# Doubiiu/ToonCrafter

Hardware: AMD Instinct MI355X
Metric: interpolated frames/sec, 512x320x16f DDIM-50 (higher is better)
Workload: dtype bf16; 1 GPU; ToonCrafter_512 320x512x16f ddim_steps=50 CFG 7.5 bf16, 1 clip per GPU (BASELINE.json configs[1]); sampler + 16f decode + 14f re-decode + splice; a different clip every step; parallelism=dp1 (independent clips, one RCCL gather)

## Files before the change

### include/tooncrafter_hip.h

```cpp
#ifndef TOONCRAFTER_HIP_H
#define TOONCRAFTER_HIP_H

#include <stdint.h>

#ifdef __cplusplus
extern "C" {
#endif

#define TC_ABI_VERSION 14

enum {
  TC_OK = 0,
  TC_EINVAL = -1,
  TC_EALIGN = -2,
  TC_ESHAPE = -3,
  TC_EWORKSPACE = -4
};

typedef uint16_t tc_bf16;

enum { TC_ACT_NONE = 0, TC_ACT_SILU = 1, TC_ACT_GELU = 2, TC_ACT_GEGLU = 3 };

enum {
  TC_GATHER_LINEAR = 0,
  TC_GATHER_CONV3x3 = 1,
  TC_GATHER_CONVT3 = 2
};

typedef struct TcGemmParams {
  const tc_bf16* a;
  const tc_bf16* w;
  void* c;
  const float* bias;
  const float* row_bias;
  const tc_bf16* residual;
  int32_t m, n, k;
  int32_t lda, ldw, ldc, ldr;
  int32_t ldrb;
  int32_t row_div;
  float alpha, out_scale;
  int32_t act;
  int32_t out_f32;
  int32_t gather;
  int32_t cin;
  int32_t frames;
  int32_t t_len;
  int32_t h_out, w_out;
  int32_t h_in, w_in;
  int32_t stride;
  int32_t upsample;
  int32_t pad;
  int32_t batch;
  int64_t stride_a, stride_w, stride_c;
  void* workspace;
  int64_t workspace_bytes;
  int32_t a_norm;
  float a_norm_eps;
  float* gn_part;
} TcGemmParams;

int tc_gemm_bf16(const TcGemmParams* p, void* stream);
int64_t tc_gemm_workspace(const TcGemmParams* p);
int tc_gemm_ws_eligible(const TcGemmParams* p);
int tc_gemm_gn_rows(const TcGemmParams* p);

typedef struct TcGemmMxParams {
  TcGemmParams g;
  const uint8_t* a_scale;
  const uint8_t* w_scale;
  int32_t lda_s, ldw_s;
} TcGemmMxParams;
int tc_gemm_mxfp8(const TcGemmMxParams* p, void* stream);
int tc_quant_mxfp8(const tc_bf16* x, int64_t rows, int32_t k, int32_t ld, uint8_t* q, int32_t ldq,
                   uint8_t* s, int32_t lds, void* stream);
int tc_layernorm_mxfp8(const tc_bf16* x, uint8_t* q, int32_t ldq, uint8_t* s, int32_t lds, const float* gamma,
                       const float* beta, int32_t rows, int32_t c, float eps, void* stream);

typedef struct TcFfParams {
  const tc_bf16* x; const tc_bf16* w1; const float* b1; const tc_bf16* w2; const float* b2; tc_bf16* out;
  int32_t m, c, hidden, ldx, ldo, ln;
  float ln_eps;
} TcFfParams;
int tc_ff_geglu_fused_eligible(const TcFfParams* p);
int tc_ff_geglu_fused(const TcFfParams* p, void* stream);

typedef struct TcTbParams {
  const tc_bf16* x; const tc_bf16* wqkv; const float* bqkv; const tc_bf16* wo; const float* bo; tc_bf16* out;
  int32_t b, t, hw, c, heads, ldx, ldo, ln;
  float ln_eps, scale;
} TcTbParams;
int tc_temporal_attn_fused_eligible(const TcTbParams* p);
int tc_temporal_attn_fused(const TcTbParams* p, void* stream);

typedef struct TcTqaParams {
  const tc_bf16* x; const tc_bf16* wqkv; const float* bqkv; tc_bf16* out;
  int32_t b, t, hw, c, heads, ldx, ldo;
  float scale;
} TcTqaParams;
int tc_temporal_qkv_attn_eligible(const TcTqaParams* p);
int tc_temporal_qkv_attn(const TcTqaParams* p, void* stream);

typedef struct TcAttnParams {
  const tc_bf16* q; const tc_bf16* k; const tc_bf16* v; tc_bf16* o;
  int32_t batch, heads, lq, lk;
  int64_t q_sb, k_sb, v_sb, o_sb;
  int32_t q_ss, k_ss, v_ss, o_ss;
  int32_t kv_bdiv;
  int32_t accumulate;
  float scale;
  const tc_bf16* k2; const tc_bf16* v2;
  int32_t lk2, kv2_bdiv;
  int64_t k2_sb, v2_sb;
  int32_t k2_ss, v2_ss;
} TcAttnParams;

int tc_attn_d64(const TcAttnParams* p, void* stream);

typedef struct TcAttnQ8Params {
  const tc_bf16* q; const tc_bf16* k; const tc_bf16* v; tc_bf16* o;
  int32_t batch, heads, lq, lk;
  int64_t q_sb, k_sb, v_sb, o_sb;
  int32_t q_ss, k_ss, v_ss, o_ss;
  float scale;
  void* workspace;
  int64_t workspace_bytes;
} TcAttnQ8Params;
int64_t tc_attn_q8_workspace(const TcAttnQ8Params* p);
int tc_attn_q8_quant_kv(const TcAttnQ8Params* p, void* stream);
int tc_attn_d64_q8(const TcAttnQ8Params* p, void* stream);

#define TC_TEMPORAL_MAX_FRAMES 64
int tc_attn_temporal(const tc_bf16* qkv, tc_bf16* out, int32_t b, int32_t t, int32_t hw,
                     int32_t heads, float scale, void* stream);

int64_t tc_groupnorm_workspace(int32_t samples, int32_t rows, int32_t c);
int tc_groupnorm(const tc_bf16* x, tc_bf16* y, const float* gamma, const float* beta,
                 int32_t samples, int32_t rows, int32_t c, float eps, int32_t silu,
                 void* workspace, int64_t workspace_bytes, void* stream);
int tc_groupnorm_part(const tc_bf16* x, tc_bf16* y, const float* gamma, const float* beta, const float* part,
                      int32_t part_rows, int32_t samples, int32_t rows, int32_t c, float eps, int32_t silu,
                      void* workspace, int64_t workspace_bytes, void* stream);


int tc_layernorm(const tc_bf16* x, tc_bf16* y, const float* gamma, const float* beta,
                 int32_t rows, int32_t c, float eps, void* stream);

#define TC_PREFETCH_MAX 4
typedef struct TcPrefetch {
  const void* ptr[TC_PREFETCH_MAX];
  int64_t bytes[TC_PREFETCH_MAX];
  int32_t n;
} TcPrefetch;
int tc_groupnorm_pf(const tc_bf16* x, tc_bf16* y, const float* gamma, const float* beta,
                    int32_t samples, int32_t rows, int32_t c, float eps, int32_t silu,
                    void* workspace, int64_t workspace_bytes, const TcPrefetch* prefetch, void* stream);
int tc_layernorm_pf(const tc_bf16* x, tc_bf16* y, const float* gamma, const float* beta,
                    int32_t rows, int32_t c, float eps, const TcPrefetch* prefetch, void* stream);

int tc_softmax_rows(const float* s, tc_bf16* p, int32_t rows, int32_t n, int32_t n_out, int32_t lds, int32_t ldo,
                    int32_t causal_period, void* stream);

int tc_nchw_to_rows(const float* x0, int32_t c0, const float* x1, int32_t c1, tc_bf16* out,
                    int32_t c_pad, int32_t b, int32_t t, int32_t hw, float scale, void* stream);
int tc_rows_to_nchw(const void* src, int32_t src_f32, int32_t ld, float* out, int32_t c,
                    int32_t b, int32_t t, int32_t hw, void* stream);
int tc_concat_rows(const tc_bf16* a, int32_t ca, const tc_bf16* b, int32_t cb, tc_bf16* out,
                   int64_t rows, void* stream);

int tc_timestep_embedding(const float* t, tc_bf16* out, int32_t n, int32_t dim, int32_t ld, void* stream);
int tc_silu_f32_to_bf16(const float* x, tc_bf16* y, int64_t n, void* stream);
int tc_timestep_embedding_i64(const int64_t* t, tc_bf16* out, int32_t n, int32_t dim, int32_t ld, void* stream);

int tc_repeat_rows(const void* src, void* dst, int64_t rows, int32_t row_bytes, int32_t n, void* stream);

int tc_time_mix3(const float* rows, int32_t ld, const float* w, const float* bias, float* out,
                 int32_t b, int32_t t, int32_t hw, void* stream);

int tc_video_to_u8(const float* x, uint8_t* out, int32_t b, int32_t t, int32_t hw, void* stream);

typedef struct TcDdimParams {
  const float* x;
  const float* e_cond;
  const float* e_uncond;
  const float* noise;
  float* x_prev; float* pred_x0;
  int32_t b; int64_t n;
  float cfg_scale, guidance_rescale;
  float sqrt_ac, sqrt_1m_ac, sqrt_a_prev, dir_coef , sigma, x0_rescale;
  const float* e_uncond_img;
  float cfg_img;
} TcDdimParams;

int64_t tc_ddim_workspace(int32_t b);
int tc_ddim_step(const TcDdimParams* p, void* workspace, int64_t workspace_bytes, void* stream);

int tc_ddim_step_eps(const TcDdimParams* p, void* workspace, int64_t workspace_bytes, void* stream);

typedef struct TcDdimBlendParams {
  const float* x;
  const float* x0;
  const float* noise;
  const float* mask;
  float* out;
  int32_t b; int64_t n;
  float sqrt_ac, sqrt_1m_ac;
} TcDdimBlendParams;
int tc_ddim_blend(const TcDdimBlendParams* p, void* stream);

int tc_abi_version(void);
const char* tc_build_info(void);

// ... 5 lines not shown
```

### tooncrafter_amd/_lib.py

```python
from __future__ import annotations

import ctypes as C
import os

HERE = os.path.dirname(os.path.abspath(__file__))
LIB_PATH = os.path.join(HERE, "libtooncrafter_hip.so")

TC_ABI_VERSION = 14
TC_TEMPORAL_MAX_FRAMES = 64
ACT_NONE, ACT_SILU, ACT_GELU, ACT_GEGLU = 0, 1, 2, 3
GATHER_LINEAR, GATHER_CONV3x3, GATHER_CONVT3 = 0, 1, 2

ERRORS = {-1: "TC_EINVAL (null pointer / bad size)", -2: "TC_EALIGN (16-byte alignment)",
          -3: "TC_ESHAPE (unsupported shape)", -4: "TC_EWORKSPACE (workspace too small)"}


class TcGemmParams(C.Structure):
    _fields_ = [
        ("a", C.c_void_p), ("w", C.c_void_p), ("c", C.c_void_p),
        ("bias", C.c_void_p), ("row_bias", C.c_void_p), ("residual", C.c_void_p),
        ("m", C.c_int32), ("n", C.c_int32), ("k", C.c_int32),
        ("lda", C.c_int32), ("ldw", C.c_int32), ("ldc", C.c_int32), ("ldr", C.c_int32),
        ("ldrb", C.c_int32), ("row_div", C.c_int32),
        ("alpha", C.c_float), ("out_scale", C.c_float),
        ("act", C.c_int32), ("out_f32", C.c_int32),
        ("gather", C.c_int32), ("cin", C.c_int32), ("frames", C.c_int32), ("t_len", C.c_int32),
        ("h_out", C.c_int32), ("w_out", C.c_int32), ("h_in", C.c_int32), ("w_in", C.c_int32),
        ("stride", C.c_int32), ("upsample", C.c_int32), ("pad", C.c_int32),
        ("batch", C.c_int32),
        ("stride_a", C.c_int64), ("stride_w", C.c_int64), ("stride_c", C.c_int64),
        ("workspace", C.c_void_p), ("workspace_bytes", C.c_int64),
        ("a_norm", C.c_int32), ("a_norm_eps", C.c_float),
        ("gn_part", C.c_void_p),
    ]


class TcGemmMxParams(C.Structure):
    _fields_ = [("g", TcGemmParams), ("a_scale", C.c_void_p), ("w_scale", C.c_void_p),
                ("lda_s", C.c_int32), ("ldw_s", C.c_int32)]


class TcAttnParams(C.Structure):
    _fields_ = [
        ("q", C.c_void_p), ("k", C.c_void_p), ("v", C.c_void_p), ("o", C.c_void_p),
        ("batch", C.c_int32), ("heads", C.c_int32), ("lq", C.c_int32), ("lk", C.c_int32),
        ("q_sb", C.c_int64), ("k_sb", C.c_int64), ("v_sb", C.c_int64), ("o_sb", C.c_int64),
        ("q_ss", C.c_int32), ("k_ss", C.c_int32), ("v_ss", C.c_int32), ("o_ss", C.c_int32),
        ("kv_bdiv", C.c_int32), ("accumulate", C.c_int32), ("scale", C.c_float),
        ("k2", C.c_void_p), ("v2", C.c_void_p), ("lk2", C.c_int32), ("kv2_bdiv", C.c_int32),
        ("k2_sb", C.c_int64), ("v2_sb", C.c_int64), ("k2_ss", C.c_int32), ("v2_ss", C.c_int32),
    ]


class TcAttnQ8Params(C.Structure):
    _fields_ = [
        ("q", C.c_void_p), ("k", C.c_void_p), ("v", C.c_void_p), ("o", C.c_void_p),
        ("batch", C.c_int32), ("heads", C.c_int32), ("lq", C.c_int32), ("lk", C.c_int32),
        ("q_sb", C.c_int64), ("k_sb", C.c_int64), ("v_sb", C.c_int64), ("o_sb", C.c_int64),
        ("q_ss", C.c_int32), ("k_ss", C.c_int32), ("v_ss", C.c_int32), ("o_ss", C.c_int32),
        ("scale", C.c_float),
        ("workspace", C.c_void_p), ("workspace_bytes", C.c_int64),
    ]


class TcDdimParams(C.Structure):
    _fields_ = [
        ("x", C.c_void_p), ("e_cond", C.c_void_p), ("e_uncond", C.c_void_p), ("noise", C.c_void_p),
        ("x_prev", C.c_void_p), ("pred_x0", C.c_void_p),
        ("b", C.c_int32), ("n", C.c_int64),
        ("cfg_scale", C.c_float), ("guidance_rescale", C.c_float),
        ("sqrt_ac", C.c_float), ("sqrt_1m_ac", C.c_float), ("sqrt_a_prev", C.c_float),
        ("dir_coef", C.c_float), ("sigma", C.c_float), ("x0_rescale", C.c_float),
        ("e_uncond_img", C.c_void_p), ("cfg_img", C.c_float),
    ]


class TcDdimBlendParams(C.Structure):
    _fields_ = [
        ("x", C.c_void_p), ("x0", C.c_void_p), ("noise", C.c_void_p), ("mask", C.c_void_p), ("out", C.c_void_p),
        ("b", C.c_int32), ("n", C.c_int64),
        ("sqrt_ac", C.c_float), ("sqrt_1m_ac", C.c_float),
    ]


class TcFfParams(C.Structure):
    _fields_ = [
# ... 21 lines not shown
    ]


TC_PREFETCH_MAX = 4


class TcPrefetch(C.Structure):
    _fields_ = [("ptr", C.c_void_p * TC_PREFETCH_MAX), ("bytes", C.c_int64 * TC_PREFETCH_MAX), ("n", C.c_int32)]


SYMBOLS = {
    "tc_gemm_bf16": (C.c_int, [C.POINTER(TcGemmParams), C.c_void_p]),
    "tc_gemm_workspace": (C.c_int64, [C.POINTER(TcGemmParams)]),
    "tc_gemm_mxfp8": (C.c_int, [C.POINTER(TcGemmMxParams), C.c_void_p]),
    "tc_quant_mxfp8": (C.c_int, [C.c_void_p, C.c_int64, C.c_int32, C.c_int32, C.c_void_p, C.c_int32, C.c_void_p, C.c_int32,
                                 C.c_void_p]),
    "tc_layernorm_mxfp8": (C.c_int, [C.c_void_p, C.c_void_p, C.c_int32, C.c_void_p, C.c_int32, C.c_void_p, C.c_void_p,
                                     C.c_int32, C.c_int32, C.c_float, C.c_void_p]),
    "tc_attn_d64": (C.c_int, [C.POINTER(TcAttnParams), C.c_void_p]),
    "tc_attn_q8_workspace": (C.c_int64, [C.POINTER(TcAttnQ8Params)]),
    "tc_attn_q8_quant_kv": (C.c_int, [C.POINTER(TcAttnQ8Params), C.c_void_p]),
    "tc_attn_d64_q8": (C.c_int, [C.POINTER(TcAttnQ8Params), C.c_void_p]),
    "tc_attn_temporal": (C.c_int, [C.c_void_p, C.c_void_p, C.c_int32, C.c_int32, C.c_int32, C.c_int32,
                                   C.c_float, C.c_void_p]),
    "tc_groupnorm_workspace": (C.c_int64, [C.c_int32, C.c_int32, C.c_int32]),
    "tc_groupnorm": (C.c_int, [C.c_void_p, C.c_void_p, C.c_void_p, C.c_void_p, C.c_int32, C.c_int32, C.c_int32,
                               C.c_float, C.c_int32, C.c_void_p, C.c_int64, C.c_void_p]),
    "tc_layernorm": (C.c_int, [C.c_void_p, C.c_void_p, C.c_void_p, C.c_void_p, C.c_int32, C.c_int32, C.c_float,
                               C.c_void_p]),
    "tc_groupnorm_pf": (C.c_int, [C.c_void_p, C.c_void_p, C.c_void_p, C.c_void_p, C.c_int32, C.c_int32, C.c_int32,
                                  C.c_float, C.c_int32, C.c_void_p, C.c_int64, C.POINTER(TcPrefetch), C.c_void_p]),
    "tc_layernorm_pf": (C.c_int, [C.c_void_p, C.c_void_p, C.c_void_p, C.c_void_p, C.c_int32, C.c_int32, C.c_float,
                                  C.POINTER(TcPrefetch), C.c_void_p]),
    "tc_softmax_rows": (C.c_int, [C.c_void_p, C.c_void_p, C.c_int32, C.c_int32, C.c_int32, C.c_int32, C.c_int32,
                                  C.c_int32, C.c_void_p]),
    "tc_nchw_to_rows": (C.c_int, [C.c_void_p, C.c_int32, C.c_void_p, C.c_int32, C.c_void_p, C.c_int32, C.c_int32,
                                  C.c_int32, C.c_int32, C.c_float, C.c_void_p]),
    "tc_rows_to_nchw": (C.c_int, [C.c_void_p, C.c_int32, C.c_int32, C.c_void_p, C.c_int32, C.c_int32, C.c_int32,
                                  C.c_int32, C.c_void_p]),
    "tc_concat_rows": (C.c_int, [C.c_void_p, C.c_int32, C.c_void_p, C.c_int32, C.c_void_p, C.c_int64, C.c_void_p]),
    "tc_timestep_embedding": (C.c_int, [C.c_void_p, C.c_void_p, C.c_int32, C.c_int32, C.c_int32, C.c_void_p]),
    "tc_silu_f32_to_bf16": (C.c_int, [C.c_void_p, C.c_void_p, C.c_int64, C.c_void_p]),
    "tc_timestep_embedding_i64": (C.c_int, [C.c_void_p, C.c_void_p, C.c_int32, C.c_int32, C.c_int32, C.c_void_p]),
    "tc_repeat_rows": (C.c_int, [C.c_void_p, C.c_void_p, C.c_int64, C.c_int32, C.c_int32, C.c_void_p]),
    "tc_time_mix3": (C.c_int, [C.c_void_p, C.c_int32, C.c_void_p, C.c_void_p, C.c_void_p, C.c_int32, C.c_int32,
                               C.c_int32, C.c_void_p]),
    "tc_video_to_u8": (C.c_int, [C.c_void_p, C.c_void_p, C.c_int32, C.c_int32, C.c_int32, C.c_void_p]),
    "tc_ddim_workspace": (C.c_int64, [C.c_int32]),
    "tc_ddim_step": (C.c_int, [C.POINTER(TcDdimParams), C.c_void_p, C.c_int64, C.c_void_p]),
    "tc_ddim_step_eps": (C.c_int, [C.POINTER(TcDdimParams), C.c_void_p, C.c_int64, C.c_void_p]),
    "tc_ddim_blend": (C.c_int, [C.POINTER(TcDdimBlendParams), C.c_void_p]),
    "tc_gemm_ws_eligible": (C.c_int, [C.POINTER(TcGemmParams)]),
    "tc_gemm_gn_rows": (C.c_int, [C.POINTER(TcGemmParams)]),
    "tc_groupnorm_part": (C.c_int, [C.c_void_p, C.c_void_p, C.c_void_p, C.c_void_p, C.c_void_p, C.c_int32, C.c_int32, C.c_int32,
                                    C.c_int32, C.c_float, C.c_int32, C.c_void_p, C.c_int64, C.c_void_p]),
    "tc_ff_geglu_fused_eligible": (C.c_int, [C.POINTER(TcFfParams)]),
    "tc_ff_geglu_fused": (C.c_int, [C.POINTER(TcFfParams), C.c_void_p]),
    "tc_temporal_attn_fused_eligible": (C.c_int, [C.POINTER(TcTbParams)]),
    "tc_temporal_attn_fused": (C.c_int, [C.POINTER(TcTbParams), C.c_void_p]),
    "tc_temporal_qkv_attn_eligible": (C.c_int, [C.POINTER(TcTqaParams)]),
    "tc_temporal_qkv_attn": (C.c_int, [C.POINTER(TcTqaParams), C.c_void_p]),
    "tc_abi_version": (C.c_int, []),
    "tc_build_info": (C.c_char_p, []),
}

_lib = None


class TooncrafterHipError(RuntimeError):
    pass


class TooncrafterAbiError(TooncrafterHipError):
    """A library built against another ABI version was loaded: a stale build, never a reason to fall back."""


def load():
    global _lib
    if _lib is not None:
        return _lib
    if not os.path.exists(LIB_PATH):
        raise TooncrafterHipError(
            f"{LIB_PATH} not found: build it with `python -m tooncrafter_amd.build` "
            "(hipcc --offload-arch=gfx950). There is no fallback path.")
    lib = C.CDLL(LIB_PATH)
    for name, (res, args) in SYMBOLS.items():
        fn = getattr(lib, name)
        fn.restype = res
        fn.argtypes = args
    ver = lib.tc_abi_version()
    if ver != TC_ABI_VERSION:
        raise TooncrafterHipError(f"ABI mismatch: library {ver}, binding {TC_ABI_VERSION}")
    if os.environ.get("TC_DEBUG_SYNC"):
        lib = _TracedLib(lib)
    _lib = lib
    return lib


class _TracedLib:

    def __init__(self, lib):
        self._lib = lib

    def __getattr__(self, name):
        fn = getattr(self._lib, name)
        if name not in SYMBOLS or name in ("tc_abi_version", "tc_build_info") or name.endswith("_workspace"):
# ... 31 lines not shown
```

### tooncrafter_amd/csrc/gemm.hip

```cpp
#include "gemm_common.h"
#include "gemm_epilogue.h"

#include <stdio.h>

namespace {

constexpr int BK = TC_BK;

template <int GATHER, int TM, int TN, bool PIPE>
__global__ __launch_bounds__(256, 2) void gemm_kernel(const TcGemmParams pin, const int splits, const int order,
                                                      const int late_epi) {
  TcGemmParams p = pin;
  if (splits > 1) {
    p.c = reinterpret_cast<float*>(pin.workspace) + (int64_t)blockIdx.y * pin.m * pin.n;
    p.ldc = pin.n;
    p.out_f32 = 1;
    p.bias = nullptr; p.row_bias = nullptr; p.residual = nullptr;
    p.act = TC_ACT_NONE; p.alpha = 1.f; p.out_scale = 1.f;
  }
  constexpr int BM = 64 * TM, BN = 64 * TN;
  constexpr int STAGE_BYTES = (BM + BN) * BK * 2;
  constexpr int EPI_BYTES = BM * BN * 4;
  constexpr int SMEM_BYTES = 2 * STAGE_BYTES > EPI_BYTES ? 2 * STAGE_BYTES : EPI_BYTES;
  constexpr int RA = BM / 32, RB = BN / 32;
  __shared__ __attribute__((aligned(1024))) char smem[SMEM_BYTES];

  const int tid = threadIdx.x;
  const int lane = tid & 63;
  const int wave = tid >> 6;
  const int wm = wave >> 1, wn = wave & 1;
  const int wave_u = __builtin_amdgcn_readfirstlane(wave);

  const int tiles_n = (p.n + BN - 1) / BN;
  const int tiles_m = (p.m + BM - 1) / BM;
  int tile_m, tile_n;
  tc_tile_of_block(blockIdx.x, tiles_m, tiles_n, order, tile_m, tile_n);
  if (tile_m >= tiles_m) return;

  const int64_t bz = blockIdx.z;
  const tc_rsrc_t w_rsrc = make_rsrc(reinterpret_cast<const bf16_t*>(p.w) + bz * p.stride_w, tc_w_extent(p));

  const int lrow = tid >> 3;
  const int chunk = (tid & 7) ^ ((lrow >> 1) & 7);
  AGather<GATHER, RA> ag;
  ag.init(p, tile_m * BM, lrow, 32, chunk);
  const tc_rsrc_t a_rsrc = tc_a_rsrc(p, bz, ag.row_lo);
  uint32_t b_voff[RB];
#pragma unroll
  for (int i = 0; i < RB; ++i) {
    const int n = tile_n * BN + lrow + 32 * i;
    b_voff[i] = n < p.n ? (uint32_t)((int64_t)n * p.ldw * 2 + chunk * 16) : TC_OOB;
  }
  const bool k_ragged = (p.k & (BK - 1)) != 0;
#if defined(TC_ABLATE) && (TC_ABLATE & 2)
  const int kb_first = blockIdx.y * (((p.k + BK - 1) / BK + splits - 1) / splits);
#endif

  auto load_tile = [&](int kb, int stage) {
#if defined(TC_ABLATE) && (TC_ABLATE & 2)
    if (kb >= kb_first + 2) return;
#endif
    const int k0 = kb * BK;
    uint32_t a_voff[RA], a_soff;
    ag.offsets(p, k0, chunk, a_voff, a_soff);
    const uint32_t kill = (k_ragged && (k0 + chunk * 8 >= p.k)) ? TC_OOB : 0u;
    char* sa = smem + stage * STAGE_BYTES + wave_u * 1024;
    char* sb = sa + BM * BK * 2;
#pragma unroll
    for (int i = 0; i < RB; ++i)
      glds16(w_rsrc, sb + i * 4096, b_voff[i] | kill, (uint32_t)k0 * 2u);
#pragma unroll
    for (int i = 0; i < RA; ++i)
      glds16(a_rsrc, sa + i * 4096, a_voff[i] | kill, a_soff);
  };

  f32x16 acc[TM][TN];
#pragma unroll
  for (int i = 0; i < TM; ++i)
#pragma unroll
    for (int j = 0; j < TN; ++j)
#pragma unroll
      for (int r = 0; r < 16; ++r) acc[i][j][r] = 0.f;

  const int frow = lane & 31;
  const int fhalf = lane >> 5;

  auto compute = [&](int stage) {
    const char* sa = smem + stage * STAGE_BYTES;
    const char* sb = sa + BM * BK * 2;
    bf16x8 af[2][TM], bf[2][TN];
    auto frags = [&](int kk, bf16x8 (&a)[TM], bf16x8 (&b)[TN]) {
      const int c = kk * 2 + fhalf;
#pragma unroll
      for (int i = 0; i < TM; ++i)
        a[i] = *reinterpret_cast<const bf16x8*>(sa + lds_off(wm * 32 * TM + i * 32 + frow, c));
#pragma unroll
      for (int j = 0; j < TN; ++j)
        b[j] = *reinterpret_cast<const bf16x8*>(sb + lds_off(wn * 32 * TN + j * 32 + frow, c));
    };
    auto mfmas = [&](bf16x8 (&a)[TM], bf16x8 (&b)[TN]) {
#if defined(TC_ABLATE) && (TC_ABLATE & 1)
      asm volatile("" ::"v"(a[0]), "v"(b[0]));
      return;
#endif
#pragma unroll
      for (int i = 0; i < TM; ++i)
#pragma unroll
        for (int j = 0; j < TN; ++j)
          acc[i][j] = __builtin_amdgcn_mfma_f32_32x32x16_bf16(a[i], b[j], acc[i][j], 0, 0, 0);
    };
    frags(0, af[0], bf[0]);
    frags(1, af[1], bf[1]);
    __builtin_amdgcn_sched_barrier(0);
    mfmas(af[0], bf[0]);
    __builtin_amdgcn_sched_barrier(0);
    frags(2, af[0], bf[0]);
    __builtin_amdgcn_sched_barrier(0);
    mfmas(af[1], bf[1]);
    __builtin_amdgcn_sched_barrier(0);
    frags(3, af[1], bf[1]);
    __builtin_amdgcn_sched_barrier(0);
    mfmas(af[0], bf[0]);
    mfmas(af[1], bf[1]);
// ... 83 lines not shown
    }
  }
  else if (p.alpha == 1.f && p.out_scale == 1.f && p.act == TC_ACT_NONE && !p.row_bias)
    epilogue_fast<false, BM, BN, true>(p, cs, tid, tile_m, tile_n, bz, pre);
  else epilogue_fast<false, BM, BN, false>(p, cs, tid, tile_m, tile_n, bz, pre);
}

__global__ __launch_bounds__(256) void splitk_reduce_kernel(const TcGemmParams p, const int splits) {
  const int vpr = p.n >> 3;
  const int64_t v = (int64_t)blockIdx.x * 256 + threadIdx.x;
  if (v >= (int64_t)p.m * vpr) return;
  const int m = (int)(v / vpr), n0 = (int)(v - (int64_t)m * vpr) * 8;
  const float* ws = reinterpret_cast<const float*>(p.workspace) + (int64_t)m * p.n + n0;
  float x[8] = {0.f, 0.f, 0.f, 0.f, 0.f, 0.f, 0.f, 0.f};
  for (int s = 0; s < splits; ++s) {
    const f32x4 lo = *reinterpret_cast<const f32x4*>(ws + (int64_t)s * p.m * p.n);
    const f32x4 hi = *reinterpret_cast<const f32x4*>(ws + (int64_t)s * p.m * p.n + 4);
#pragma unroll
    for (int e = 0; e < 4; ++e) { x[e] += lo[e]; x[4 + e] += hi[e]; }
  }
#pragma unroll
  for (int e = 0; e < 8; ++e) {
    float t = x[e] * p.alpha;
    if (p.bias) t += p.bias[n0 + e];
    if (p.row_bias) t += p.row_bias[(int64_t)(m / p.row_div) * p.ldrb + n0 + e];
    x[e] = apply_act(t, p.act) * p.out_scale;
  }
  if (p.residual) {
    float rf[8];
    unpack8(*reinterpret_cast<const u32x4*>(reinterpret_cast<const bf16_t*>(p.residual) + (int64_t)m * p.ldr + n0), rf);
#pragma unroll
    for (int e = 0; e < 8; ++e) x[e] += rf[e];
  }
  if (p.out_f32) {
    float* op = reinterpret_cast<float*>(p.c) + (int64_t)m * p.ldc + n0;
    *reinterpret_cast<f32x4*>(op) = f32x4{x[0], x[1], x[2], x[3]};
    *reinterpret_cast<f32x4*>(op + 4) = f32x4{x[4], x[5], x[6], x[7]};
  } else {
    *reinterpret_cast<u32x4*>(reinterpret_cast<bf16_t*>(p.c) + (int64_t)m * p.ldc + n0) = pack8(x);
  }
}

}

static void tc_gemm_tile_launch(const TcGemmParams& p, const TcGemmRoute& r, hipStream_t s) {
  const dim3 grid(r.grid[0], r.grid[1], r.grid[2]), block(r.block);
  const auto go = [&](auto g, auto pipe) {
    constexpr int G = decltype(g)::value, P = decltype(pipe)::value;
    if (r.tm == 2 && r.tn == 2) hipLaunchKernelGGL((gemm_kernel<G, 2, 2, P>), grid, block, 0, s, p, r.splits, r.order, r.late_epi);
    else if (r.tm == 2) hipLaunchKernelGGL((gemm_kernel<G, 2, 1, P>), grid, block, 0, s, p, r.splits, r.order, r.late_epi);
    else if (r.tn == 2) hipLaunchKernelGGL((gemm_kernel<G, 1, 2, P>), grid, block, 0, s, p, r.splits, r.order, r.late_epi);
    else hipLaunchKernelGGL((gemm_kernel<G, 1, 1, P>), grid, block, 0, s, p, r.splits, r.order, r.late_epi);
  };
  tc_with_gather(p.gather, [&](auto g) { if (r.pipe) go(g, std::true_type{}); else go(g, std::false_type{}); });
}

extern "C" int tc_gemm_bf16(const TcGemmParams* pp, void* stream) {
  if (!pp) return TC_EINVAL;
  const TcGemmParams& p = *pp;
  if (const int rc = tc_gemm_validate(p)) return rc;
  const int cus = tc_cu_count();
  const TcGemmSwitches sw = tc_gemm_switches();
  TcGemmRoute r;
  const int rc = tc_gemm_route(p, sw, cus, &r);
  static bool said = false;
  if (r.halo_yielded && !said) {
    said = true;
    fprintf(stderr, "[tooncrafter_hip] %s=%s is set: the 3x3 convolutions stay on the implicit-GEMM kernels "
                    "(halo-patch route suppressed; TC_CONV_HALO=2 forces it)\n", sw.forcing_name, sw.forcing_value);
  }
  if (rc != TC_OK) return rc;
  static TcGemmLaunch* const launch[] = {tc_gemm_ws_launch, tc_conv_halo_launch, tc_gemm8_launch, tc_gemm_tile16_launch,
                                         tc_gemm_wide_launch, tc_gemm_tile_launch};
  launch[r.family](p, r, reinterpret_cast<hipStream_t>(stream));
  TC_LAUNCH_CHECK();
  if (r.family == TC_FAM_TILE && r.splits > 1) {
    const int64_t vecs = (int64_t)p.m * (p.n >> 3);
    hipLaunchKernelGGL(splitk_reduce_kernel, dim3((unsigned)((vecs + 255) / 256)), dim3(256), 0, reinterpret_cast<hipStream_t>(stream), p, r.splits);
    TC_LAUNCH_CHECK();
  }
  return TC_OK;
}
```

### tooncrafter_amd/csrc/gemm_mx.hip

```cpp
#include "gemm_common.h"
#include "gemm_epilogue.h"
#include "mx_quant.h"

namespace {

constexpr int BKE = 128;
typedef int i32x8 __attribute__((ext_vector_type(8)));
typedef int i32x4 __attribute__((ext_vector_type(4)));

template <int GATHER, int R>
struct MxRows {
  uint32_t base[R];
  uint32_t vbits[R];
  int f[R], y[R], x[R];
  bool ok[R];

  __device__ __forceinline__ void init(const TcGemmParams& p, int ld, int row0, int row_step) {
    const int hw = p.h_out * p.w_out;
#pragma unroll
    for (int i = 0; i < R; ++i) {
      const int mm = row0 + row_step * i;
      ok[i] = mm < p.m;
      const int mc = ok[i] ? mm : 0;
      f[i] = y[i] = x[i] = 0;
// ... 248 lines not shown
  const u32x4* src = reinterpret_cast<const u32x4*>(x + row * ld + blk * 32);
  u32x4 v[4];
#pragma unroll
  for (int i = 0; i < 4; ++i) v[i] = src[i];
  uint32_t amax = 0;
#pragma unroll
  for (int i = 0; i < 4; ++i)
#pragma unroll
    for (int e = 0; e < 4; ++e) {
      const uint32_t lo = v[i][e] & 0x7fffu, hi = (v[i][e] >> 16) & 0x7fffu;
      amax = max(amax, max(lo, hi));
    }
  const int byte = mx_scale_byte(amax);
  const float inv = mx_inv_scale(byte);
  uint32_t out[8];
#pragma unroll
  for (int i = 0; i < 4; ++i) {
    float f[8];
    unpack8(v[i], f);
    out[i * 2] = mx_quant4(f[0], f[1], f[2], f[3], inv);
    out[i * 2 + 1] = mx_quant4(f[4], f[5], f[6], f[7], inv);
  }
  u32x4* dst = reinterpret_cast<u32x4*>(q + row * ldq + blk * 32);
  dst[0] = u32x4{out[0], out[1], out[2], out[3]};
  dst[1] = u32x4{out[4], out[5], out[6], out[7]};
  s[slot] = (uint8_t)byte;
}

}

extern "C" int tc_quant_mxfp8(const tc_bf16* x, int64_t rows, int32_t k, int32_t ld, uint8_t* q, int32_t ldq,
                              uint8_t* s, int32_t lds, void* stream) {
  if (!x || !q || !s || rows <= 0 || k <= 0) return TC_EINVAL;
  if ((k & 31) || (ld & 7) || (ldq & 15) || !tc_aligned16(x) || !tc_aligned16(q)) return TC_EALIGN;
  if (ld < k || ldq < k || lds * 32 < k) return TC_ESHAPE;
  const int64_t slots = rows * lds;
  if ((slots + 255) / 256 > 0x7fffffffLL) return TC_ESHAPE;
  hipLaunchKernelGGL(quant_mx_kernel, dim3((unsigned)((slots + 255) / 256)), dim3(256), 0, reinterpret_cast<hipStream_t>(stream),
                     reinterpret_cast<const bf16_t*>(x), rows, k, ld, q, ldq, s, lds);
  TC_LAUNCH_CHECK();
  return TC_OK;
}

extern "C" int tc_gemm_mxfp8(const TcGemmMxParams* pp, void* stream) {
  if (!pp) return TC_EINVAL;
  const TcGemmParams& p = pp->g;
  if (!p.a || !p.w || !p.c || !pp->a_scale || !pp->w_scale || p.m <= 0 || p.n <= 0 || p.k <= 0) return TC_EINVAL;
  if (!tc_aligned16(p.a) || !tc_aligned16(p.w) || !tc_aligned16(p.c)) return TC_EALIGN;
  if (p.residual && !tc_aligned16(p.residual)) return TC_EALIGN;
  if ((p.k & 31) || (p.lda & 15) || (p.ldw & 15)) return TC_EALIGN;
  if ((reinterpret_cast<uintptr_t>(pp->a_scale) & 1u) || (reinterpret_cast<uintptr_t>(pp->w_scale) & 3u)) return TC_EALIGN;
  if ((pp->lda_s & 1) || (pp->ldw_s & 3)) return TC_EALIGN;
  if (p.ldw < p.k || pp->ldw_s < ((p.k + 127) / 128) * 4) return TC_ESHAPE;
  if ((p.batch > 1) || p.stride_a || p.stride_w || p.stride_c) return TC_ESHAPE;
  const bool geglu = p.act == TC_ACT_GEGLU;
  const int n_out = geglu ? p.n / 2 : p.n;
  if ((n_out & 7) == 0) {
    if (p.out_f32 ? (p.ldc & 3) : (p.ldc & 7)) return TC_EALIGN;
    if (p.residual && (p.ldr & 7)) return TC_EALIGN;
    if (p.bias && (reinterpret_cast<uintptr_t>(p.bias) & 15u)) return TC_EALIGN;
    if (p.row_bias && ((reinterpret_cast<uintptr_t>(p.row_bias) & 15u) || (p.ldrb & 3))) return TC_EALIGN;
  }
  if (p.ldc < n_out || (p.residual && p.ldr < n_out)) return TC_ESHAPE;
  if (geglu && ((p.n % 128) != 0 || p.row_bias || p.residual)) return TC_ESHAPE;
  if (p.row_bias && (p.row_div <= 0 || p.ldrb < p.n)) return TC_EINVAL;
  if (p.act < TC_ACT_NONE || p.act > TC_ACT_GEGLU) return TC_EINVAL;
  if (p.gather == TC_GATHER_LINEAR) {
    if (p.lda < p.k || pp->lda_s < ((p.k + 63) / 64) * 2) return TC_ESHAPE;
  } else if (p.gather == TC_GATHER_CONV3x3 || p.gather == TC_GATHER_CONVT3) {
    const int taps = p.gather == TC_GATHER_CONV3x3 ? 9 : 3;
    if (p.cin <= 0 || (p.cin % 64) != 0 || p.k != taps * p.cin || p.lda < p.cin || pp->lda_s * 32 < p.cin) return TC_ESHAPE;
    if ((int64_t)p.k * p.cin >= (1LL << 32)) return TC_ESHAPE;
    if (p.frames <= 0 || p.h_out <= 0 || p.w_out <= 0) return TC_ESHAPE;
    if ((int64_t)p.frames * p.h_out * p.w_out != p.m) return TC_ESHAPE;
    if (p.gather == TC_GATHER_CONV3x3) {
      if (p.h_in <= 0 || p.w_in <= 0 || (p.stride != 1 && p.stride != 2)) return TC_ESHAPE;
      if (p.upsample && p.stride != 1) return TC_ESHAPE;
      const int hvv = p.upsample ? 2 * p.h_in : p.h_in, wvv = p.upsample ? 2 * p.w_in : p.w_in;
      if (p.pad != 0 && p.pad != 1) return TC_ESHAPE;
      const int extra = p.pad == 1 ? 2 : 1;
      if ((hvv + extra - 3) / p.stride + 1 != p.h_out || (wvv + extra - 3) / p.stride + 1 != p.w_out) return TC_ESHAPE;
    } else {
      if (p.t_len <= 0 || (p.frames % p.t_len) != 0) return TC_ESHAPE;
    }
  } else {
    return TC_EINVAL;
  }
  if (tc_a_rows(p) * p.lda >= 0x7fffff00LL || (int64_t)p.n * p.ldw >= 0x7fffff00LL) return TC_ESHAPE;
  hipStream_t s = reinterpret_cast<hipStream_t>(stream);
  const int64_t big_tiles = (int64_t)((p.n + 127) / 128) * ((p.m + 127) / 128);
  const bool small = !geglu && big_tiles < 384;
  const int bm = small ? 64 : 128;
  const int tiles_n = (p.n + bm - 1) / bm;
  const int tiles_m = (p.m + bm - 1) / bm;
  const int64_t nblk = (int64_t)tiles_n * 8 * ((tiles_m + 7) / 8);
  if (nblk > 0x7fffffffLL) return TC_ESHAPE;
  dim3 grid((unsigned)nblk), block(256);
  TcGemmParams half = p;
  half.ldw = p.ldw / 2;
  const int order = tc_gemm_tile_order(half, tiles_n, tc_gemm_switches());
#define TC_LAUNCH_MX(G)                                                                            \
  do {                                                                                             \
    if (small) hipLaunchKernelGGL((gemm_mx_kernel<G, 1, 1>), grid, block, 0, s, *pp, order);        \
    else hipLaunchKernelGGL((gemm_mx_kernel<G, 2, 2>), grid, block, 0, s, *pp, order);              \
  } while (0)
  switch (p.gather) {
    case TC_GATHER_LINEAR: TC_LAUNCH_MX(TC_GATHER_LINEAR); break;
// ... 8 lines not shown
```

### tooncrafter_amd/csrc/gemm_route.cpp

```cpp
#include "gemm_route.h"

#include <stdlib.h>
#include <string.h>

namespace {

typedef TcGemmSwitches S;
const struct Sw { const char* name; const char* dflt; bool implicit_gemm; char kind; int S::*field; } kSwitches[] = {
    {"TC_GEMM_TILE", nullptr, false, 't', &S::tile},
    {"TC_GEMM_TILE16", "1", true, 'i', &S::tile16},
    {"TC_GEMM8", "1", true, 'i', &S::gemm8},
    {"TC_GEMM_PIPE", "1", true, 'p', &S::pipe},
    {"TC_GEMM_SPLITK", nullptr, true, 'k', &S::splitk},
    {"TC_GEMM_WS", "1", true, 'i', &S::ws},
    {"TC_G16_ILV", nullptr, true, 'l', &S::ilv},
    {"TC_G16_TALL", "0", true, 'i', &S::g16_tall},
    {"TC_GEMM_WIDE", "1", true, '0', &S::wide},
    {"TC_GEMM_ORDER", "8", true, 'i', &S::order},
    {"TC_GEMM_NMAJOR", "1", true, 'i', &S::nmajor},
    {"TC_GEMM_ORDER_MIB", "4", false, 'm', nullptr},
    {"TC_GEMM_EPI_LATE", "0", false, '1', &S::epi_late},
    {"TC_G8_GRID", "0", false, 'i', &S::g8_grid},
    {"TC_G8_STAGGER", "0", false, 'i', &S::g8_stagger},
    {"TC_CONV_HALO", "1", false, 'i', &S::halo},
// ... 8 lines not shown

void take(TcGemmRoute* r, int family, int64_t gx, int gy, int gz, int block) {
  r->family = family, r->block = (unsigned)block;
  r->grid[0] = (unsigned)gx, r->grid[1] = (unsigned)gy, r->grid[2] = (unsigned)gz;
}

}

TcGemmSwitches tc_gemm_switches() {
  TcGemmSwitches s{};
  for (const Sw& sw : kSwitches) {
    const char* e = getenv(sw.name);
    const char* v = e ? e : sw.dflt;
    if (sw.implicit_gemm && !s.forcing_name && e && e[0] && !(sw.dflt && strcmp(e, sw.dflt) == 0)) s.forcing_name = sw.name, s.forcing_value = e;
    if (sw.kind == 'i') s.*sw.field = atoi(v);
    else if (sw.kind == '0') s.*sw.field = v[0] != '0';
    else if (sw.kind == '1') s.*sw.field = v[0] == '1';
    else if (sw.kind == 'p') s.pipe = v[0] == '0' ? 0 : v[0] == '2' ? 2 : 1;
    else if (sw.kind == 'k') s.splitk = e ? atoi(e) : -1;
    else if (sw.kind == 'l') s.ilv_set = e != nullptr, s.ilv = e ? atoi(e) : 0;
    else if (sw.kind == 'm') s.order_bytes = (int64_t)(atof(v) * (1 << 20));
    else if (e) {
      const int t = e[0] == 'w' ? 1 : e[0] == 'b' ? 22 : e[0] == 's' ? 11 : atoi(e);
      s.tile = (t == 22 || t == 21 || t == 12 || t == 11 || e[0] == 'w') ? t : 0, s.tile_set = e[0] != 0;
    }
  }
  static const TcGemmSwitches first = s;
  s.order = first.order, s.order_bytes = first.order_bytes;
  return s;
}

int tc_gemm_tile_order(const TcGemmParams& p, int tiles_n, const TcGemmSwitches& sw) {
  return (sw.order > 0 && tiles_n >= 2 * sw.order && (int64_t)p.n * p.ldw * 2 > sw.order_bytes) ? sw.order : 0;
}

int tc_gemm_validate(const TcGemmParams& p) {
  if (!p.a || !p.w || !p.c || p.m <= 0 || p.n <= 0 || p.k <= 0) return TC_EINVAL;
  if (!aligned16(p.a) || !aligned16(p.w) || !aligned16(p.c)) return TC_EALIGN;
  if (p.residual && !aligned16(p.residual)) return TC_EALIGN;
  if ((p.k & 7) || (p.lda & 7) || (p.ldw & 7)) return TC_EALIGN;
  if (p.ldw < p.k) return TC_ESHAPE;
  const bool geglu = p.act == TC_ACT_GEGLU;
  const int n_out = geglu ? p.n / 2 : p.n;
  if ((n_out & 7) == 0) {
    if (p.out_f32 ? (p.ldc & 3) : (p.ldc & 7)) return TC_EALIGN;
    if (p.residual && (p.ldr & 7)) return TC_EALIGN;
    if (p.bias && !aligned16(p.bias)) return TC_EALIGN;
    if (p.row_bias && (!aligned16(p.row_bias) || (p.ldrb & 3))) return TC_EALIGN;
  }
  if (p.ldc < n_out || (p.residual && p.ldr < n_out)) return TC_ESHAPE;
  if (geglu && ((p.n % 128) != 0 || p.row_bias || p.residual)) return TC_ESHAPE;
  if (p.row_bias && (p.row_div <= 0 || p.ldrb < p.n)) return TC_EINVAL;
  if (p.act < TC_ACT_NONE || p.act > TC_ACT_GEGLU) return TC_EINVAL;
  if (p.gather == TC_GATHER_LINEAR) {
    if (p.lda < p.k) return TC_ESHAPE;
  } else if (p.gather == TC_GATHER_CONV3x3 || p.gather == TC_GATHER_CONVT3) {
    const int taps = p.gather == TC_GATHER_CONV3x3 ? 9 : 3;
    if (p.cin <= 0 || (p.cin % 64) != 0 || p.k != taps * p.cin || p.lda < p.cin) return TC_ESHAPE;
    if (p.frames <= 0 || p.h_out <= 0 || p.w_out <= 0) return TC_ESHAPE;
    if ((int64_t)p.frames * p.h_out * p.w_out != p.m) return TC_ESHAPE;
    if (p.gather == TC_GATHER_CONV3x3) {
      if (p.h_in <= 0 || p.w_in <= 0 || (p.stride != 1 && p.stride != 2)) return TC_ESHAPE;
      if (p.upsample && p.stride != 1) return TC_ESHAPE;
      const int hvv = p.upsample ? 2 * p.h_in : p.h_in, wvv = p.upsample ? 2 * p.w_in : p.w_in;
      if (p.pad != 0 && p.pad != 1) return TC_ESHAPE;
      const int extra = p.pad == 1 ? 2 : 1;
      if ((hvv + extra - 3) / p.stride + 1 != p.h_out || (wvv + extra - 3) / p.stride + 1 != p.w_out) return TC_ESHAPE;
    } else {
      if (p.t_len <= 0 || (p.frames % p.t_len) != 0) return TC_ESHAPE;
    }
  } else {
    return TC_EINVAL;
  }
  int64_t span_rows = 256;
  if (p.gather == TC_GATHER_CONVT3) span_rows += 2 * (int64_t)p.h_out * p.w_out;
  else if (p.gather == TC_GATHER_CONV3x3)
    span_rows = ((int64_t)256 / (p.w_out > 0 ? p.w_out : 1) + 2) * p.stride * p.w_in + 4 * (int64_t)p.w_in + 8;
  const int64_t a_bytes = (span_rows + 1) * p.lda * 2, w_bytes = (int64_t)p.n * p.ldw * 2;
  return (a_bytes < 0x7fffff00LL && w_bytes < 0x7fffff00LL) ? TC_OK : TC_ESHAPE;
}

static bool tc_gemm_ws_takes(const TcGemmParams& p, const TcGemmSwitches& sw, int batch) {
  if (sw.tile_set) return false;
  if (sw.ws == 0 || batch != 1 || p.gather != TC_GATHER_LINEAR || p.k != TC_WS_K || p.lda < TC_WS_K) return false;
  if (p.row_bias || p.alpha != 1.f || p.out_scale != 1.f || p.out_f32) return false;
  const bool geglu = p.act == TC_ACT_GEGLU;
  if (!geglu && p.act != TC_ACT_NONE) return false;
  if (p.n % (geglu ? 256 : 320) != 0) return false;
  if (p.residual && geglu) return false;
  if ((sw.ws == 1 || sw.ws == 5) && (p.m < 65536 || geglu || p.n != 320)) return false;
  if ((int64_t)p.m * p.lda * 2 >= 0x7fffff00LL) return false;
  if ((int64_t)p.m * p.ldc * 2 >= 0x7fffff00LL || (p.residual && (int64_t)p.m * p.ldr * 2 >= 0x7fffff00LL)) return false;
  return true;
}

static void route_ws(const TcGemmParams& p, const TcGemmSwitches& sw, TcGemmRoute* r) {
  r->geglu = p.act == TC_ACT_GEGLU, r->res = p.residual != nullptr, r->ln = p.a_norm != 0;
  const int slabs = p.n / (r->geglu ? 256 : 320);
  const int ntiles = (p.m + TC_WS_ROWS - 1) / TC_WS_ROWS;
  int nchunks = 256 / slabs < 1 ? 1 : 256 / slabs;
  r->nchunks = nchunks = nchunks > ntiles ? ntiles : nchunks;
  r->safe = sw.ws == 3 ? 1 : (sw.ws == 2 ? 0 : 2);
  take(r, TC_FAM_WS, slabs * 8 * ((nchunks + 7) / 8), 1, 1, 256);
}

static int route_halo(const TcGemmParams& p, const TcGemmSwitches& sw, int batch, TcGemmRoute* r) {
  if (sw.halo == 0) return 0;
// ... 133 lines not shown
  const int force = sw.splitk;
  const int batch = p.batch > 0 ? p.batch : 1;
  if (force == 0 || batch != 1 || p.act == TC_ACT_GEGLU || (p.n & 7) != 0) return 1;
  const int nk = (p.k + TC_BK - 1) / TC_BK;
  const int64_t tiles = (int64_t)((p.n + 127) / 128) * ((p.m + 127) / 128);
  if (tiles >= 200 || (force < 0 && nk < 128)) return 1;
  int s = force > 0 ? force : (int)(512 / tiles);
  if (s > 8) s = 8;
  if (s > nk / 8) s = nk / 8;
  if (force <= 0) while (s & (s - 1)) s &= s - 1;
  return s < 2 ? 1 : s;
}

static void pick_tile(int m, int n, int batch, bool geglu, int* tm, int* tn) {
  const int64_t big_tiles = (int64_t)((n + 127) / 128) * ((m + 127) / 128) * batch;
  const bool small = !geglu && big_tiles < 384;
  *tm = small ? 1 : 2;
  *tn = small ? 1 : 2;
  if (!geglu && n <= 64) {
    *tn = 1;
    *tm = m >= 262144 ? 2 : 1;
  }
}

static int route_tile(const TcGemmParams& p, const TcGemmSwitches& sw, int batch, bool gn_ok, TcGemmRoute* r) {
  const bool geglu = p.act == TC_ACT_GEGLU;
  const int force = sw.tile;
  int tm = 2, tn = 2;
  int splits = (p.workspace && force == 0) ? tc_gemm_splits(p, sw) : 1;
  if (splits > 1 && p.workspace_bytes < (int64_t)splits * p.m * p.n * (int64_t)sizeof(float)) splits = 1;
  if (force > 1) {
    tm = force / 10;
    tn = geglu ? 2 : force % 10;
  } else if (splits == 1) {
    pick_tile(p.m, p.n, batch, geglu, &tm, &tn);
  }
  r->gn_rows = (gn_ok && splits == 1 && tm == 2 && tn == 2) ? 128 : 0;
  if (p.gn_part && !r->gn_rows) return TC_ESHAPE;
  if (splits > 1 && !aligned16(p.workspace)) return TC_EALIGN;
  const int bm = 64 * tm, bn = 64 * tn;
  const int tiles_n = (p.n + bn - 1) / bn;
  const int tiles_m = (p.m + bm - 1) / bm;
  const bool nmajor = sw.nmajor != 0 && p.batch <= 1 && (sw.nmajor == 2 || (p.m <= 2048 && tc_w_extent(p) > tc_a_extent(p)));
  const int64_t nblk = nmajor ? 8 * (((int64_t)tiles_m * tiles_n + 7) / 8) : (int64_t)tiles_n * 8 * ((tiles_m + 7) / 8);
  if (nblk > 0x7fffffffLL || batch > 65535) return TC_ESHAPE;
  take(r, TC_FAM_TILE, nblk, splits, batch, 256);
  r->tm = tm, r->tn = tn, r->splits = splits;
  r->order = nmajor ? -1 : tc_gemm_tile_order(p, tiles_n, sw);
  r->pipe = sw.pipe != 0, r->late_epi = sw.epi_late;
  return TC_OK;
}

int tc_gemm_route(const TcGemmParams& p, const TcGemmSwitches& sw, int cus, TcGemmRoute* r) {
  *r = TcGemmRoute{};
  const int batch = p.batch > 0 ? p.batch : 1;
  const bool gn_ok = batch == 1 && p.act != TC_ACT_GEGLU && !p.out_f32 && (p.n & 7) == 0 && !p.a_norm && !sw.tile_set && sw.gn_part;
  if (p.gn_part && !gn_ok) return TC_ESHAPE;
  const auto emits = [&](int rows) {
    r->gn_rows = gn_ok ? rows : 0;
    return (p.gn_part && !r->gn_rows) ? TC_ESHAPE : TC_OK;
  };
  const int force = sw.tile;
  if (force == 0 && tc_gemm_ws_takes(p, sw, batch)) return route_ws(p, sw, r), emits(0);
  if (p.a_norm) return TC_ESHAPE;
  if (force == 0 && !p.gn_part) {
    const int h = route_halo(p, sw, batch, r);
    if (h < 0) return TC_ESHAPE;
    if (h > 0) return TC_OK;
  }
  if (force == 0 && route_gemm8(p, sw, batch, cus, r)) return emits(0);
  if (force == 0 && route_tile16(p, sw, batch, r)) return emits(TC_T16);
  if (force <= 1 && route_wide(p, sw, batch, force == 1, r)) return emits(0);
  return route_tile(p, sw, batch, gn_ok, r);
}

extern "C" int64_t tc_gemm_workspace(const TcGemmParams* p) {
  if (!p || p->m <= 0 || p->n <= 0 || p->k <= 0) return 0;
  const int s = tc_gemm_splits(*p, tc_gemm_switches());
  return s > 1 ? (int64_t)s * p->m * p->n * (int64_t)sizeof(float) : 0;
}
extern "C" int tc_gemm_ws_eligible(const TcGemmParams* p) {
  return (p && tc_gemm_ws_takes(*p, tc_gemm_switches(), p->batch > 0 ? p->batch : 1)) ? 1 : 0;
}

extern "C" int tc_gemm_gn_rows(const TcGemmParams* pp) {
  if (!pp || pp->m <= 0 || pp->n <= 0 || pp->k <= 0) return 0;
  TcGemmParams p = *pp;
  if (!p.gn_part) p.gn_part = reinterpret_cast<float*>(16);
  TcGemmRoute r;
  tc_gemm_route(p, tc_gemm_switches(), 256, &r);
  return r.gn_rows;
}
```

### tooncrafter_amd/csrc/norm.hip

```cpp
#include "common.h"
#include "mx_quant.h"

#include <stdlib.h>

namespace {

constexpr int GN_THREADS = 256;
constexpr int GN_MAX_SLOTS = 2;
constexpr int GN_TARGET_BLOCKS = 512;
constexpr int GN_MIN_ROWS = 8;

constexpr int PF_MAX = 4;
struct PfArgs {
  const u32x4* p[PF_MAX];
  uint32_t units[PF_MAX];
  int n;
};

__device__ __forceinline__ void pf_run(const PfArgs& pf, uint32_t b, uint32_t nb, uint32_t tid, uint32_t nthr) {
#pragma unroll 1
  for (int i = 0; i < pf.n; ++i) {
    const u32x4* src = pf.p[i];
    const uint32_t units = pf.units[i];
    uint32_t per = (units + nb - 1) / nb;
    per = (per + 7u) & ~7u;
    const uint32_t lo = b * per;
    if (lo >= units) continue;
    const uint32_t hi = min(units, lo + per);
#pragma unroll 1
    for (uint32_t u = lo + tid; u < hi; u += nthr * 16u) {
      u32x4 v[16];
#pragma unroll
      for (int k = 0; k < 16; ++k) {
        const uint32_t uu = u + (uint32_t)k * nthr;
        v[k] = uu < hi ? src[uu] : u32x4{0u, 0u, 0u, 0u};
      }
#pragma unroll
      for (int k = 0; k < 16; ++k) asm volatile("" ::"v"(v[k][0]), "v"(v[k][1]), "v"(v[k][2]), "v"(v[k][3]));
    }
  }
}

struct GnGeo {
  int vpr;
  int slots;
  int rows_pp;
};

__host__ __device__ __forceinline__ GnGeo gn_geo(int c) {
  GnGeo g;
  g.vpr = c >> 3;
  g.slots = (g.vpr + GN_THREADS - 1) / GN_THREADS;
  const int vps = (g.vpr + g.slots - 1) / g.slots;
  g.rows_pp = g.slots > 1 ? 1 : GN_THREADS / vps;
  if (g.rows_pp < 1) g.rows_pp = 1;
  return g;
}

__device__ __forceinline__ void gn_thread_map(const GnGeo& g, int tid, int& rlane, int (&vec)[GN_MAX_SLOTS]) {
  if (g.slots > 1) {
    rlane = 0;
#pragma unroll
    for (int s = 0; s < GN_MAX_SLOTS; ++s) {
      const int v = tid + s * GN_THREADS;
      vec[s] = (s < g.slots && v < g.vpr) ? v : -1;
    }
  } else {
    rlane = tid / g.vpr;
    vec[0] = rlane < g.rows_pp ? tid - rlane * g.vpr : -1;
    if (rlane >= g.rows_pp) rlane = 0;
    vec[1] = -1;
  }
}

__global__ __launch_bounds__(GN_THREADS) void gn_stats_kernel(const bf16_t* __restrict__ x, float* __restrict__ part,
                                                              int rows, int c, int nchunks, int chunk_rows) {
  __shared__ float red[2][4096 + 32];
  const GnGeo g = gn_geo(c);
  const int tid = threadIdx.x;
  int rlane, vec[GN_MAX_SLOTS];
  gn_thread_map(g, tid, rlane, vec);
  const int sample = blockIdx.y, chunk = blockIdx.x;
  const int r0 = chunk * chunk_rows;
  const int r1 = min(rows, r0 + chunk_rows);
  const bf16_t* xs = x + (int64_t)sample * rows * c;

  float sum[GN_MAX_SLOTS][8], sq[GN_MAX_SLOTS][8];
#pragma unroll
  for (int s = 0; s < GN_MAX_SLOTS; ++s)
#pragma unroll
    for (int e = 0; e < 8; ++e) { sum[s][e] = 0.f; sq[s][e] = 0.f; }

  const int step = g.rows_pp;
  for (int r = r0 + rlane; r < r1; r += 4 * step) {
#pragma unroll
    for (int s = 0; s < GN_MAX_SLOTS; ++s) {
      if (vec[s] >= 0) {
        u32x4 v4[4];
#pragma unroll
        for (int u = 0; u < 4; ++u) {
          const int rr = r + u * step;
          v4[u] = rr < r1 ? *reinterpret_cast<const u32x4*>(xs + (int64_t)rr * c + vec[s] * 8)
                          : u32x4{0u, 0u, 0u, 0u};
        }
#pragma unroll
        for (int u = 0; u < 4; ++u) {
          float f[8];
          unpack8(v4[u], f);
#pragma unroll
          for (int e = 0; e < 8; ++e) { sum[s][e] += f[e]; sq[s][e] += f[e] * f[e]; }
        }
      }
    }
  }
  for (int pass = 0; pass < g.rows_pp; ++pass) {
    if (rlane == pass) {
#pragma unroll
      for (int s = 0; s < GN_MAX_SLOTS; ++s)
        if (vec[s] >= 0) {
#pragma unroll
          for (int e = 0; e < 8; ++e) {
            const int ch = vec[s] * 8 + e;
            if (pass == 0) { red[0][ch] = sum[s][e]; red[1][ch] = sq[s][e]; }
            else { red[0][ch] += sum[s][e]; red[1][ch] += sq[s][e]; }
          }
        }
    }
    __syncthreads();
  }
  if (tid < 32) {
    const int cpg = c / 32;
    float a = 0.f, b = 0.f;
    for (int i = 0; i < cpg; ++i) { a += red[0][tid * cpg + i]; b += red[1][tid * cpg + i]; }
    float* o = part + (((int64_t)sample * nchunks + chunk) * 32 + tid) * 2;
    o[0] = a;
    o[1] = b;
  }
}

__global__ __launch_bounds__(256) void gn_finalize_kernel(const float* __restrict__ part, float* __restrict__ stats,
                                                          int samples, int rows, int c, int nchunks, float eps) {
  const int lane = threadIdx.x & 63;
  const int sg = blockIdx.x * 4 + (threadIdx.x >> 6);
  if (sg >= samples * 32) return;
  const int sample = sg >> 5, grp = sg & 31;
  const float* pp = part + ((int64_t)sample * nchunks * 32 + grp) * 2;
  double a = 0.0, b = 0.0;
  for (int k = lane; k < nchunks; k += 64) {
    const float2 v = *reinterpret_cast<const float2*>(pp + (int64_t)k * 64);
    a += v.x;
    b += v.y;
  }
#pragma unroll
  for (int off = 32; off > 0; off >>= 1) { a += __shfl_xor(a, off, 64); b += __shfl_xor(b, off, 64); }
  if (lane == 0) {
    const double cnt = (double)rows * (c / 32);
    const double mean = a / cnt;
    double var = b / cnt - mean * mean;
    if (var < 0.0) var = 0.0;
    stats[(int64_t)sg * 2] = (float)mean;
    stats[(int64_t)sg * 2 + 1] = (float)(1.0 / sqrt(var + (double)eps));
  }
}

__global__ __launch_bounds__(256) void gn_finalize_part_kernel(const float* __restrict__ part, float* __restrict__ stats,
                                                               int samples, int rows, int c, int prows, float eps) {
  __shared__ double red[2][4];
  const int tid = threadIdx.x, lane = tid & 63, wave = tid >> 6;
  const int sg = blockIdx.x;
  const int sample = sg >> 5, grp = sg & 31;
  const int cpg = c / 32, nb = rows / prows;
  const float* pp = part + ((int64_t)sample * nb * 2) * c + grp * cpg;
  double a = 0.0, b = 0.0;
  for (int blk = tid; blk < nb; blk += 256) {
    const float* r0 = pp + (int64_t)blk * 2 * c;
    for (int ch = 0; ch < cpg; ++ch) { a += r0[ch]; b += r0[c + ch]; }
  }
#pragma unroll
  for (int off = 32; off > 0; off >>= 1) { a += __shfl_xor(a, off, 64); b += __shfl_xor(b, off, 64); }
  if (lane == 0) { red[0][wave] = a; red[1][wave] = b; }
  __syncthreads();
  if (tid == 0) {
    a = red[0][0] + red[0][1] + red[0][2] + red[0][3];
    b = red[1][0] + red[1][1] + red[1][2] + red[1][3];
    const double cnt = (double)rows * cpg;
    const double mean = a / cnt;
    double var = b / cnt - mean * mean;
    if (var < 0.0) var = 0.0;
    stats[(int64_t)sg * 2] = (float)mean;
    stats[(int64_t)sg * 2 + 1] = (float)(1.0 / sqrt(var + (double)eps));
  }
}

template <bool SILU>
__global__ __launch_bounds__(GN_THREADS) void gn_apply_kernel(const bf16_t* __restrict__ x, bf16_t* __restrict__ y,
                                                              const float* __restrict__ gamma, const float* __restrict__ beta,
                                                              const float* __restrict__ stats, int rows, int c,
                                                              int chunk_rows, const PfArgs pf) {
  if (blockIdx.z) {
    pf_run(pf, ((blockIdx.z - 1) * gridDim.y + blockIdx.y) * gridDim.x + blockIdx.x, (gridDim.z - 1) * gridDim.y * gridDim.x,
           threadIdx.x, GN_THREADS);
    return;
  }
  const GnGeo g = gn_geo(c);
  const int tid = threadIdx.x;
  int rlane, vec[GN_MAX_SLOTS];
  gn_thread_map(g, tid, rlane, vec);
  const int sample = blockIdx.y, chunk = blockIdx.x;
  const float* st = stats + (int64_t)sample * 64;
  const int cpg = c / 32;
  float sc[GN_MAX_SLOTS][8], sh[GN_MAX_SLOTS][8];
#pragma unroll
  for (int s = 0; s < GN_MAX_SLOTS; ++s)
#pragma unroll
    for (int e = 0; e < 8; ++e) {
      sc[s][e] = 0.f; sh[s][e] = 0.f;
      if (vec[s] >= 0) {
        const int ch = vec[s] * 8 + e;
        const int grp = ch / cpg;
        const float a = st[grp * 2 + 1] * gamma[ch];
        sc[s][e] = a;
        sh[s][e] = beta[ch] - st[grp * 2] * a;
      }
    }
  const int r0 = chunk * chunk_rows;
  const int r1 = min(rows, r0 + chunk_rows);
  const bf16_t* xs = x + (int64_t)sample * rows * c;
  bf16_t* ys = y + (int64_t)sample * rows * c;
  const int step = g.rows_pp;
  for (int r = r0 + rlane; r < r1; r += 4 * step) {
#pragma unroll
    for (int s = 0; s < GN_MAX_SLOTS; ++s) {
      if (vec[s] >= 0) {
        u32x4 v4[4];
#pragma unroll
        for (int u = 0; u < 4; ++u) {
          const int rr = r + u * step;
          if (rr < r1) v4[u] = *reinterpret_cast<const u32x4*>(xs + (int64_t)rr * c + vec[s] * 8);
        }
#pragma unroll
        for (int u = 0; u < 4; ++u) {
          const int rr = r + u * step;
          if (rr < r1) {
            float f[8];
            unpack8(v4[u], f);
#pragma unroll
            for (int e = 0; e < 8; ++e) {
              const float v = f[e] * sc[s][e] + sh[s][e];
              f[e] = SILU ? silu_f(v) : v;
            }
            *reinterpret_cast<u32x4*>(ys + (int64_t)rr * c + vec[s] * 8) = pack8(f);
          }
        }
      }
    }
  }
}

__device__ __forceinline__ void gn_opaque(u32x4& v) { asm volatile("" : "+v"(v[0]), "+v"(v[1]), "+v"(v[2]), "+v"(v[3])); }

template <int T, int NV, bool SILU>
__global__ __launch_bounds__(T) void gn_onepass_kernel(const bf16_t* __restrict__ x, bf16_t* __restrict__ y,
                                                       const float* __restrict__ gamma, const float* __restrict__ beta,
                                                       int rows, int c, int vu, float eps, const PfArgs pf) {
  if (blockIdx.z) {
    pf_run(pf, ((blockIdx.z - 1) * gridDim.y + blockIdx.y) * gridDim.x + blockIdx.x, (gridDim.z - 1) * gridDim.y * gridDim.x,
           threadIdx.x, T);
    return;
  }
  constexpr int NW = T / 64;
  __shared__ float red[2][NW][4];
  const int tid = threadIdx.x, lane = tid & 63, wave = tid >> 6;
  const int cpg = c >> 5;
  const int rpp = T / vu;
  const int col = tid % vu, r0 = tid / vu;
  const bool live = tid < rpp * vu;
  const int unit = blockIdx.x, sample = blockIdx.y;
  const int ch0 = (unit * vu + col) * 8;
  const int ug0 = (unit * vu * 8) / cpg;
  const bf16_t* xs = x + (int64_t)sample * rows * c + ch0;
  bf16_t* ys = y + (int64_t)sample * rows * c + ch0;
  int gl[8];
#pragma unroll
  for (int e = 0; e < 8; ++e) gl[e] = (ch0 + e) / cpg - ug0;

  u32x4 v[NV];
#pragma unroll
  for (int i = 0; i < NV; ++i) {
    const int r = r0 + i * rpp;
    v[i] = (live && r < rows) ? *reinterpret_cast<const u32x4*>(xs + (int64_t)r * c) : u32x4{0u, 0u, 0u, 0u};
  }
  auto group_sums = [&](const float (&pc)[8], int slot, float (&out)[4]) {
    float g4[4] = {0.f, 0.f, 0.f, 0.f};
#pragma unroll
    for (int e = 0; e < 8; ++e)
#pragma unroll
      for (int g = 0; g < 4; ++g) g4[g] += (gl[e] == g) ? pc[e] : 0.f;
#pragma unroll
    for (int g = 0; g < 4; ++g) g4[g] = wave_sum(g4[g]);
    if (lane == 0) {
#pragma unroll
      for (int g = 0; g < 4; ++g) red[slot][wave][g] = g4[g];
    }
    __syncthreads();
#pragma unroll
    for (int g = 0; g < 4; ++g) {
      float t = 0.f;
#pragma unroll
      for (int w = 0; w < NW; ++w) t += red[slot][w][g];
      out[g] = t;
    }
  };
  float pc[8] = {0.f, 0.f, 0.f, 0.f, 0.f, 0.f, 0.f, 0.f};
#pragma unroll
  for (int i = 0; i < NV; ++i) {
    float f[8];
    unpack8(v[i], f);
#pragma unroll
    for (int e = 0; e < 8; ++e) pc[e] += f[e];
  }
  float gs[4];
  group_sums(pc, 0, gs);
  const float inv_cnt = 1.0f / ((float)rows * (float)cpg);
  float mean_e[8];
#pragma unroll
  for (int e = 0; e < 8; ++e) {
    float m = 0.f;
#pragma unroll
    for (int g = 0; g < 4; ++g) m = (gl[e] == g) ? gs[g] * inv_cnt : m;
    mean_e[e] = m;
  }
#pragma unroll
  for (int e = 0; e < 8; ++e) pc[e] = 0.f;
#pragma unroll
  for (int i = 0; i < NV; ++i) {
    const int r = r0 + i * rpp;
    gn_opaque(v[i]);
    if (live && r < rows) {
      float f[8];
      unpack8(v[i], f);
#pragma unroll
      for (int e = 0; e < 8; ++e) { const float d = f[e] - mean_e[e]; pc[e] += d * d; }
    }
// ... 154 lines not shown
static int pf_args(const TcPrefetch* pf, PfArgs* out) {
  PfArgs a{};
  a.n = 0;
  if (pf) {
    if (pf->n < 0 || pf->n > TC_PREFETCH_MAX) return TC_EINVAL;
    for (int i = 0; i < pf->n; ++i) {
      if (!pf->ptr[i] || pf->bytes[i] < 0 || pf->bytes[i] > ((int64_t)1 << 35)) return TC_EINVAL;
      if (!tc_aligned16(pf->ptr[i])) return TC_EALIGN;
      const uint32_t units = (uint32_t)(pf->bytes[i] >> 4);
      if (!units) continue;
      a.p[a.n] = reinterpret_cast<const u32x4*>(pf->ptr[i]);
      a.units[a.n] = units;
      ++a.n;
    }
  }
  *out = a;
  return TC_OK;
}
static inline unsigned pf_planes(const PfArgs& a, int64_t plane) {
  if (!a.n || plane <= 0) return 0;
  int64_t z = (512 + plane - 1) / plane;
  if (z > 8) {
    int64_t units = 0;
    for (int i = 0; i < a.n; ++i) units += a.units[i];
    int64_t need = (units * 16 + 65535) / 65536;
    if (need > 512) need = 512;
    const int64_t zn = (need + plane - 1) / plane;
    z = zn > 8 ? (zn > 64 ? 64 : zn) : 8;
  }
  return (unsigned)(z < 1 ? 1 : z);
}

static inline void gn_chunking(int samples, int rows, int* nchunks, int* chunk_rows) {
  static const int target = [] { const char* e = getenv("TC_GN_BLOCKS"); const int v = e ? atoi(e) : 0;
                                 return v > 0 ? v : GN_TARGET_BLOCKS; }();
  int per_sample = target / (samples > 0 ? samples : 1);
  if (per_sample < 1) per_sample = 1;
  int max_chunks = (rows + GN_MIN_ROWS - 1) / GN_MIN_ROWS;
  int n = per_sample < max_chunks ? per_sample : max_chunks;
  if (n < 1) n = 1;
  const int cr = (rows + n - 1) / n;
  *chunk_rows = cr;
  *nchunks = (rows + cr - 1) / cr;
}

extern "C" int64_t tc_groupnorm_workspace(int32_t samples, int32_t rows, int32_t c) {
  (void)c;
  if (samples <= 0 || rows <= 0) return 0;
  int nch, cr;
  gn_chunking(samples, rows, &nch, &cr);
  return ((int64_t)samples * nch * 64 + (int64_t)samples * 64) * sizeof(float);
}

static int gn_check(const tc_bf16* x, tc_bf16* y, const float* gamma, const float* beta, int32_t samples, int32_t rows,
                    int32_t c, void* workspace, int64_t workspace_bytes, const TcPrefetch* prefetch, PfArgs* pf) {
  if (!x || !y || !gamma || !beta || !workspace || samples <= 0 || rows <= 0 || c <= 0) return TC_EINVAL;
  if (const int rc = pf_args(prefetch, pf)) return rc;
  if ((c % 32) != 0 || c > GN_MAX_SLOTS * GN_THREADS * 8 || c > 4096) return TC_ESHAPE;
  if (!tc_aligned16(x) || !tc_aligned16(y)) return TC_EALIGN;
  if (workspace_bytes < tc_groupnorm_workspace(samples, rows, c)) return TC_EWORKSPACE;
  if (samples > 65535) return TC_ESHAPE;
  return TC_OK;
}

struct GnIo {
  const bf16_t* x; bf16_t* y; const float* gamma; const float* beta;
  int rows, c; bool silu; hipStream_t s;
};
static void gn_apply_launch(const GnIo& io, dim3 grid, const float* stats, int chunk_rows, const PfArgs& pf) {
  const auto k = io.silu ? gn_apply_kernel<true> : gn_apply_kernel<false>;
  hipLaunchKernelGGL(k, grid, dim3(GN_THREADS), 0, io.s, io.x, io.y, io.gamma, io.beta, stats, io.rows, io.c, chunk_rows, pf);
}
template <int T, int NV>
static void gn_onepass_launch(const GnIo& io, dim3 grid, int vu, float eps, const PfArgs& pf) {
  const auto k = io.silu ? gn_onepass_kernel<T, NV, true> : gn_onepass_kernel<T, NV, false>;
  hipLaunchKernelGGL(k, grid, dim3(T), 0, io.s, io.x, io.y, io.gamma, io.beta, io.rows, io.c, vu, eps, pf);
}

static int groupnorm_impl(const tc_bf16* x, tc_bf16* y, const float* gamma, const float* beta,
                          int32_t samples, int32_t rows, int32_t c, float eps, int32_t silu,
                          void* workspace, int64_t workspace_bytes, const TcPrefetch* prefetch, void* stream) {
  PfArgs pf;
  if (const int rc = gn_check(x, y, gamma, beta, samples, rows, c, workspace, workspace_bytes, prefetch, &pf)) return rc;
  const GnIo io = {reinterpret_cast<const bf16_t*>(x), reinterpret_cast<bf16_t*>(y), gamma, beta, rows, c, silu != 0,
                   reinterpret_cast<hipStream_t>(stream)};
  {
    static const bool onepass = [] { const char* e = getenv("TC_GN_ONEPASS"); return !(e && e[0] == '0'); }();
    const int cpg = c / 32;
    int u = cpg;
    while (u % 8) u += cpg;
    const int vu = u / 8, gu = u / cpg;
    if (onepass && (c % u) == 0 && gu <= 4 && vu <= 64 && tc_aligned16(gamma) && tc_aligned16(beta)) {
      const int64_t nvec = (int64_t)rows * vu;
      const dim3 grid(c / u, samples, 1 + pf_planes(pf, (int64_t)(c / u) * samples));
      auto fits = [&](int t, int nv) { return (int64_t)((rows + t / vu - 1) / (t / vu)) <= nv; };
      const int64_t nblk = (int64_t)(c / u) * samples;
      const int64_t bytes = nvec * 16 * samples * (c / u);
      bool done = nblk >= 128 || bytes <= (4 << 20);
      if (done && fits(256, 4)) gn_onepass_launch<256, 4>(io, grid, vu, eps, pf);
      else if (done && fits(256, 13)) gn_onepass_launch<256, 13>(io, grid, vu, eps, pf);
      else done = false;
      if (done) {
        TC_LAUNCH_CHECK();
        return TC_OK;
      }
    }
  }
  int nch, cr;
  gn_chunking(samples, rows, &nch, &cr);
  float* part = reinterpret_cast<float*>(workspace);
  float* stats = part + (int64_t)samples * nch * 64;
  dim3 grid(nch, samples), block(GN_THREADS);
  hipLaunchKernelGGL(gn_stats_kernel, grid, block, 0, io.s, io.x, part, rows, c, nch, cr);
  TC_LAUNCH_CHECK();
  hipLaunchKernelGGL(gn_finalize_kernel, dim3((samples * 32 + 3) / 4), block, 0, io.s, part, stats, samples, rows, c, nch,
                     eps);
  TC_LAUNCH_CHECK();
  gn_apply_launch(io, dim3(nch, samples, 1 + pf_planes(pf, (int64_t)nch * samples)), stats, cr, pf);
  TC_LAUNCH_CHECK();
  return TC_OK;
}

extern "C" int tc_groupnorm(const tc_bf16* x, tc_bf16* y, const float* gamma, const float* beta,
                            int32_t samples, int32_t rows, int32_t c, float eps, int32_t silu,
                            void* workspace, int64_t workspace_bytes, void* stream) {
  return groupnorm_impl(x, y, gamma, beta, samples, rows, c, eps, silu, workspace, workspace_bytes, nullptr, stream);
}

extern "C" int tc_groupnorm_pf(const tc_bf16* x, tc_bf16* y, const float* gamma, const float* beta,
                               int32_t samples, int32_t rows, int32_t c, float eps, int32_t silu,
                               void* workspace, int64_t workspace_bytes, const TcPrefetch* prefetch, void* stream) {
  return groupnorm_impl(x, y, gamma, beta, samples, rows, c, eps, silu, workspace, workspace_bytes, prefetch, stream);
}

extern "C" int tc_groupnorm_part(const tc_bf16* x, tc_bf16* y, const float* gamma, const float* beta, const float* part,
                                 int32_t part_rows, int32_t samples, int32_t rows, int32_t c, float eps, int32_t silu,
                                 void* workspace, int64_t workspace_bytes, void* stream) {
  if (!part || part_rows <= 0) return TC_EINVAL;
  PfArgs pf;
  if (const int rc = gn_check(x, y, gamma, beta, samples, rows, c, workspace, workspace_bytes, nullptr, &pf)) return rc;
  if ((rows % part_rows) != 0) return TC_ESHAPE;
  const GnIo io = {reinterpret_cast<const bf16_t*>(x), reinterpret_cast<bf16_t*>(y), gamma, beta, rows, c, silu != 0,
                   reinterpret_cast<hipStream_t>(stream)};
  int nch, cr;
  gn_chunking(samples, rows, &nch, &cr);
  float* stats = reinterpret_cast<float*>(workspace) + (int64_t)samples * nch * 64;
  hipLaunchKernelGGL(gn_finalize_part_kernel, dim3(samples * 32), dim3(256), 0, io.s, part, stats, samples, rows, c,
                     part_rows, eps);
  TC_LAUNCH_CHECK();
  gn_apply_launch(io, dim3(nch, samples), stats, cr, pf);
  TC_LAUNCH_CHECK();
  return TC_OK;
}

template <bool MX>
static void ln_launch(const tc_bf16* x, tc_bf16* y, const float* gamma, const float* beta, int32_t rows, int32_t c, float eps,
                      uint8_t* q, int32_t ldq, uint8_t* sc, int32_t lds, const PfArgs& pf, void* stream) {
  const int rpb = c <= 512 ? 16 : (c <= 1024 ? 8 : 4);
  const unsigned blocks = (unsigned)((rows + rpb - 1) / rpb);
  const auto k = c <= 512 ? layernorm_kernel<1, 4, MX> : (c <= 1024 ? layernorm_kernel<2, 2, MX> : layernorm_kernel<4, 1, MX>);
  hipLaunchKernelGGL(k, dim3(blocks, 1 + pf_planes(pf, blocks)), dim3(256), 0, reinterpret_cast<hipStream_t>(stream),
                     reinterpret_cast<const bf16_t*>(x), reinterpret_cast<bf16_t*>(y), gamma, beta, rows, c, eps, q, ldq, sc, lds, pf);
}

static int layernorm_impl(const tc_bf16* x, tc_bf16* y, const float* gamma, const float* beta,
                          int32_t rows, int32_t c, float eps, const TcPrefetch* prefetch, void* stream) {
  if (!x || !y || !gamma || !beta || rows <= 0 || c <= 0) return TC_EINVAL;
  if ((c % 8) != 0 || c > 4 * 64 * 8) return TC_ESHAPE;
  if (!tc_aligned16(x) || !tc_aligned16(y) || !tc_aligned16(gamma) || !tc_aligned16(beta)) return TC_EALIGN;
  PfArgs pf;
  if (const int rc = pf_args(prefetch, &pf)) return rc;
  ln_launch<false>(x, y, gamma, beta, rows, c, eps, nullptr, 0, nullptr, 0, pf, stream);
  TC_LAUNCH_CHECK();
  return TC_OK;
}

extern "C" int tc_layernorm(const tc_bf16* x, tc_bf16* y, const float* gamma, const float* beta,
                            int32_t rows, int32_t c, float eps, void* stream) {
  return layernorm_impl(x, y, gamma, beta, rows, c, eps, nullptr, stream);
}

extern "C" int tc_layernorm_pf(const tc_bf16* x, tc_bf16* y, const float* gamma, const float* beta,
                               int32_t rows, int32_t c, float eps, const TcPrefetch* prefetch, void* stream) {
  return layernorm_impl(x, y, gamma, beta, rows, c, eps, prefetch, stream);
}

extern "C" int tc_layernorm_mxfp8(const tc_bf16* x, uint8_t* q, int32_t ldq, uint8_t* sc, int32_t lds, const float* gamma,
                                  const float* beta, int32_t rows, int32_t c, float eps, void* stream) {
  if (!x || !q || !sc || !gamma || !beta || rows <= 0 || c <= 0) return TC_EINVAL;
  if ((c % 32) != 0 || c > 4 * 64 * 8 || ldq < c || lds * 32 < c) return TC_ESHAPE;
  if (!tc_aligned16(x) || !tc_aligned16(gamma) || !tc_aligned16(beta) || (reinterpret_cast<uintptr_t>(q) & 7u) || (ldq & 7)) return TC_EALIGN;
  const int vpr = c >> 3, pad = lds - (c >> 5);
  const int nv = c <= 512 ? 1 : (c <= 1024 ? 2 : 4);
  if (vpr + pad > 64 * nv) return TC_ESHAPE;
  ln_launch<true>(x, nullptr, gamma, beta, rows, c, eps, q, ldq, sc, lds, PfArgs{}, stream);
  TC_LAUNCH_CHECK();
// ... 12 lines not shown
```

### tooncrafter_amd/csrc/torch_ops.cpp

```cpp
#include <ATen/ATen.h>
#include <c10/hip/HIPStream.h>
#include <torch/library.h>

#include <tuple>
#include <vector>

#include "tooncrafter_hip.h"

namespace {

using at::Tensor;
using c10::optional;

void* cur_stream() { return reinterpret_cast<void*>(c10::hip::getCurrentHIPStream().stream()); }

void check_rc(int rc, const char* what) {
  TORCH_CHECK(rc == 0, what, " failed with code ", rc,
              rc < 0 ? " (TC_E*: -1 invalid, -2 alignment, -3 unsupported shape, -4 workspace)" : " (hipError_t)");
}

const tc_bf16* bf(const Tensor& t) { return reinterpret_cast<const tc_bf16*>(t.data_ptr()); }

void check_rows(const Tensor& t, const char* name, at::ScalarType dt = at::kBFloat16) {
  TORCH_CHECK(t.is_cuda(), name, ": expected a CUDA tensor (the product path is GPU-only)");
// ... 20 lines not shown
  p.ldc = (int32_t)out.stride(0);
  p.alpha = (float)alpha; p.out_scale = (float)out_scale; p.act = (int32_t)act; p.out_f32 = out_f32 ? 1 : 0;
  p.batch = 1;
  if (bias.has_value()) {
    TORCH_CHECK(bias->is_cuda() && bias->scalar_type() == at::kFloat && bias->is_contiguous() && bias->numel() == g.n,
                "gemm: bias must be a contiguous fp32 CUDA [N]");
    p.bias = bias->data_ptr<float>();
  }
  if (row_bias.has_value()) {
    check_rows(*row_bias, "gemm: row_bias", at::kFloat);
    TORCH_CHECK(row_div > 0 && row_bias->size(1) == g.n && row_bias->size(0) * row_div >= g.m, "gemm: row_bias / row_div do not cover M");
    p.row_bias = row_bias->data_ptr<float>(); p.ldrb = (int32_t)row_bias->stride(0); p.row_div = (int32_t)row_div;
  }
  if (residual.has_value()) {
    check_rows(*residual, "gemm: residual");
    TORCH_CHECK(residual->size(1) == g.n_out && residual->size(0) >= g.m, "gemm: residual shape mismatch");
    p.residual = bf(*residual); p.ldr = (int32_t)residual->stride(0);
  }
  if (conv.empty()) {
    p.gather = TC_GATHER_LINEAR;
    TORCH_CHECK(a.size(1) >= g.k, "gemm: A has fewer columns than the weight's K");
  } else {
    p.gather = conv[0] == 1 ? TC_GATHER_CONV3x3 : TC_GATHER_CONVT3;
    p.cin = (int32_t)conv[1]; p.frames = (int32_t)conv[2]; p.t_len = (int32_t)conv[3];
    p.h_in = (int32_t)conv[4]; p.w_in = (int32_t)conv[5]; p.h_out = (int32_t)conv[6]; p.w_out = (int32_t)conv[7];
    p.stride = (int32_t)conv[8]; p.upsample = (int32_t)conv[9]; p.pad = (int32_t)conv[10];
    TORCH_CHECK(a.size(0) >= (int64_t)p.frames * p.h_in * p.w_in && a.size(1) >= p.cin, "gemm: conv source too small for its geometry");
  }
}

Tensor gemm_cuda(const Tensor& a, const Tensor& w, const optional<Tensor>& bias, const optional<Tensor>& residual,
                 const optional<Tensor>& row_bias, int64_t row_div, int64_t act, double alpha, double out_scale,
                 bool out_f32, at::IntArrayRef conv, double a_norm_eps) {
  check_rows(a, "gemm: a");
  check_rows(w, "gemm: w");
  const GemmGeom g = gemm_geom(a, w, act, conv);
  Tensor out = at::empty({g.m, g.n_out}, a.options().dtype(out_f32 ? at::kFloat : at::kBFloat16));
  TcGemmParams p = {};
  p.a = bf(a); p.w = bf(w);
  p.lda = (int32_t)a.stride(0); p.ldw = (int32_t)w.stride(0);
  fill_gemm(p, a, g, out, bias, residual, row_bias, row_div, act, alpha, out_scale, out_f32, conv);
  if (a_norm_eps >= 0.0) {
    p.a_norm = 1; p.a_norm_eps = (float)a_norm_eps;
    TORCH_CHECK(tc_gemm_ws_eligible(&p) == 1, "gemm: a_norm_eps needs a problem the weight-stationary kernel takes");
  }
  Tensor ws;
  const int64_t nbytes = tc_gemm_workspace(&p);
  if (nbytes > 0) {
    ws = at::empty({nbytes}, a.options().dtype(at::kByte));
    p.workspace = ws.data_ptr(); p.workspace_bytes = nbytes;
  }
  check_rc(tc_gemm_bf16(&p, cur_stream()), "tc_gemm_bf16");
  return out;
}

std::tuple<Tensor, Tensor> quant_mxfp8_cuda(const Tensor& x, int64_t k) {
  check_rows(x, "quant_mxfp8: x");
  TORCH_CHECK(k > 0 && k % 32 == 0 && x.size(1) >= k, "quant_mxfp8: k must be a multiple of 32 and <= the columns of x");
  const int64_t rows = x.size(0), lds = (k + 127) / 128 * 4;
  Tensor q = at::empty({rows, k}, x.options().dtype(at::kByte));
  Tensor s = at::empty({rows, lds}, x.options().dtype(at::kByte));
  check_rc(tc_quant_mxfp8(bf(x), rows, (int32_t)k, (int32_t)x.stride(0), q.data_ptr<uint8_t>(), (int32_t)q.stride(0),
                          s.data_ptr<uint8_t>(), (int32_t)lds, cur_stream()), "tc_quant_mxfp8");
  return {q, s};
}

std::tuple<Tensor, Tensor> quant_mxfp8_meta(const Tensor& x, int64_t k) {
  return {at::empty({x.size(0), k}, x.options().dtype(at::kByte)),
          at::empty({x.size(0), (k + 127) / 128 * 4}, x.options().dtype(at::kByte))};
}

Tensor gemm_mx_cuda(const Tensor& aq, const Tensor& a_scale, const Tensor& wq, const Tensor& w_scale, const optional<Tensor>& bias,
                    const optional<Tensor>& residual, const optional<Tensor>& row_bias, int64_t row_div, int64_t act,
                    double alpha, double out_scale, bool out_f32, at::IntArrayRef conv) {
  check_rows(aq, "gemm_mx: a", at::kByte); check_rows(wq, "gemm_mx: w", at::kByte);
  check_rows(a_scale, "gemm_mx: a_scale", at::kByte); check_rows(w_scale, "gemm_mx: w_scale", at::kByte);
  TORCH_CHECK(a_scale.size(0) == aq.size(0) && w_scale.size(0) == wq.size(0), "gemm_mx: one scale row per operand row");
  const GemmGeom g = gemm_geom(aq, wq, act, conv);
  Tensor out = at::empty({g.m, g.n_out}, aq.options().dtype(out_f32 ? at::kFloat : at::kBFloat16));
  TcGemmMxParams px = {};
  px.g.a = reinterpret_cast<const tc_bf16*>(aq.data_ptr()); px.g.w = reinterpret_cast<const tc_bf16*>(wq.data_ptr());
  px.g.lda = (int32_t)aq.stride(0); px.g.ldw = (int32_t)wq.stride(0);
  fill_gemm(px.g, aq, g, out, bias, residual, row_bias, row_div, act, alpha, out_scale, out_f32, conv);
  px.a_scale = a_scale.data_ptr<uint8_t>(); px.lda_s = (int32_t)a_scale.stride(0);
  px.w_scale = w_scale.data_ptr<uint8_t>(); px.ldw_s = (int32_t)w_scale.stride(0);
  check_rc(tc_gemm_mxfp8(&px, cur_stream()), "tc_gemm_mxfp8");
  return out;
}

Tensor gemm_mx_meta(const Tensor& aq, const Tensor&, const Tensor& wq, const Tensor&, const optional<Tensor>&, const optional<Tensor>&,
                    const optional<Tensor>&, int64_t, int64_t act, double, double, bool out_f32, at::IntArrayRef conv) {
  const GemmGeom g = gemm_geom(aq, wq, act, conv);
  return at::empty({g.m, g.n_out}, aq.options().dtype(out_f32 ? at::kFloat : at::kBFloat16));
}

Tensor gemm_meta(const Tensor& a, const Tensor& w, const optional<Tensor>&, const optional<Tensor>&, const optional<Tensor>&,
                 int64_t, int64_t act, double, double, bool out_f32, at::IntArrayRef conv, double) {
  const GemmGeom g = gemm_geom(a, w, act, conv);
  return at::empty({g.m, g.n_out}, a.options().dtype(out_f32 ? at::kFloat : at::kBFloat16));
}

Tensor attention_cuda(const Tensor& q, const Tensor& k, const Tensor& v, int64_t batch, int64_t heads, int64_t lq, int64_t lk,
                      int64_t kv_bdiv, double scale, const optional<Tensor>& k2, const optional<Tensor>& v2, int64_t lk2,
                      int64_t kv2_bdiv) {
  check_rows(q, "attention: q"); check_rows(k, "attention: k"); check_rows(v, "attention: v");
  const int64_t hd = heads * 64;
// ... 61 lines not shown
                            (int32_t)heads, (float)scale, cur_stream()), "tc_attn_temporal");
  return out;
}

Tensor attention_temporal_meta(const Tensor& qkv, int64_t b, int64_t t, int64_t hw, int64_t heads, double) {
  return at::empty({b * t * hw, heads * 64}, qkv.options());
}

void check_affine(const Tensor& g, const Tensor& b, int64_t c, const char* what) {
  TORCH_CHECK(g.is_cuda() && b.is_cuda() && g.scalar_type() == at::kFloat && b.scalar_type() == at::kFloat &&
              g.is_contiguous() && b.is_contiguous() && g.numel() == c && b.numel() == c, what, ": gamma / beta must be contiguous fp32 CUDA [C]");
}

Tensor groupnorm_cuda(const Tensor& x, const Tensor& gamma, const Tensor& beta, int64_t samples, int64_t rows, double eps, bool silu) {
  check_rows(x, "groupnorm: x");
  const int64_t c = x.size(1);
  TORCH_CHECK(x.is_contiguous() && x.size(0) == samples * rows, "groupnorm: x must be contiguous [samples*rows, C]");
  check_affine(gamma, beta, c, "groupnorm");
  Tensor y = at::empty_like(x);
  const int64_t nbytes = tc_groupnorm_workspace((int32_t)samples, (int32_t)rows, (int32_t)c);
  Tensor ws = at::empty({nbytes > 16 ? nbytes : 16}, x.options().dtype(at::kByte));
  check_rc(tc_groupnorm(bf(x), reinterpret_cast<tc_bf16*>(y.data_ptr()), gamma.data_ptr<float>(), beta.data_ptr<float>(),
                        (int32_t)samples, (int32_t)rows, (int32_t)c, (float)eps, silu ? 1 : 0, ws.data_ptr(), nbytes, cur_stream()),
           "tc_groupnorm");
  return y;
}

TcPrefetch prefetch_of(at::TensorList ts, const char* what) {
  TORCH_CHECK((int64_t)ts.size() <= TC_PREFETCH_MAX, what, ": at most ", TC_PREFETCH_MAX, " prefetch tensors");
  TcPrefetch pf = {};
  for (const Tensor& t : ts) {
    TORCH_CHECK(t.is_cuda() && t.is_contiguous(), what, ": prefetch tensors must be contiguous CUDA tensors");
    pf.ptr[pf.n] = t.data_ptr();
    pf.bytes[pf.n] = (int64_t)t.numel() * (int64_t)t.element_size();
    ++pf.n;
  }
  return pf;
}

Tensor groupnorm_pf_cuda(const Tensor& x, const Tensor& gamma, const Tensor& beta, int64_t samples, int64_t rows, double eps, bool silu,
                         at::TensorList prefetch) {
  check_rows(x, "groupnorm_pf: x");
  const int64_t c = x.size(1);
  TORCH_CHECK(x.is_contiguous() && x.size(0) == samples * rows, "groupnorm_pf: x must be contiguous [samples*rows, C]");
  check_affine(gamma, beta, c, "groupnorm_pf");
  const TcPrefetch pf = prefetch_of(prefetch, "groupnorm_pf");
  Tensor y = at::empty_like(x);
  const int64_t nbytes = tc_groupnorm_workspace((int32_t)samples, (int32_t)rows, (int32_t)c);
  Tensor ws = at::empty({nbytes > 16 ? nbytes : 16}, x.options().dtype(at::kByte));
  check_rc(tc_groupnorm_pf(bf(x), reinterpret_cast<tc_bf16*>(y.data_ptr()), gamma.data_ptr<float>(), beta.data_ptr<float>(),
                           (int32_t)samples, (int32_t)rows, (int32_t)c, (float)eps, silu ? 1 : 0, ws.data_ptr(), nbytes, &pf, cur_stream()),
           "tc_groupnorm_pf");
  return y;
}

Tensor layernorm_pf_cuda(const Tensor& x, const Tensor& gamma, const Tensor& beta, double eps, at::TensorList prefetch) {
  check_rows(x, "layernorm_pf: x");
  TORCH_CHECK(x.is_contiguous(), "layernorm_pf: x must be contiguous");
  check_affine(gamma, beta, x.size(1), "layernorm_pf");
  const TcPrefetch pf = prefetch_of(prefetch, "layernorm_pf");
  Tensor y = at::empty_like(x);
  check_rc(tc_layernorm_pf(bf(x), reinterpret_cast<tc_bf16*>(y.data_ptr()), gamma.data_ptr<float>(), beta.data_ptr<float>(),
                           (int32_t)x.size(0), (int32_t)x.size(1), (float)eps, &pf, cur_stream()), "tc_layernorm_pf");
  return y;
}

Tensor groupnorm_pf_meta(const Tensor& x, const Tensor&, const Tensor&, int64_t, int64_t, double, bool, at::TensorList) { return at::empty_like(x); }
Tensor layernorm_pf_meta(const Tensor& x, const Tensor&, const Tensor&, double, at::TensorList) { return at::empty_like(x); }

void check_w(const Tensor& t, at::ScalarType dt, const char* name) {
  TORCH_CHECK(t.is_cuda() && t.scalar_type() == dt && t.is_contiguous(), name, ": expected a contiguous CUDA tensor of dtype ", dt);
}

Tensor ff_geglu_fused_cuda(const Tensor& x, const Tensor& w1, const Tensor& b1, const Tensor& w2, const Tensor& b2, double ln_eps) {
  check_rows(x, "ff_geglu_fused: x");
  check_w(w1, at::kBFloat16, "ff_geglu_fused: w1"); check_w(w2, at::kBFloat16, "ff_geglu_fused: w2");
  check_w(b1, at::kFloat, "ff_geglu_fused: b1"); check_w(b2, at::kFloat, "ff_geglu_fused: b2");
  const int64_t m = x.size(0), c = x.size(1);
  TORCH_CHECK(w2.dim() == 2 && w1.dim() == 2, "ff_geglu_fused: w1 [2 hidden, c], w2 [c, hidden]");
  const int64_t hidden = w2.size(1);
  TORCH_CHECK(w1.size(0) == 2 * hidden && w1.size(1) == c && w2.size(0) == c && b1.numel() == 2 * hidden && b2.numel() == c,
              "ff_geglu_fused: x [m, c] rows, w1 [2 hidden, c], b1 [2 hidden], w2 [c, hidden], b2 [c]");
  Tensor out = at::empty({m, c}, x.options());
  TcFfParams p{};
  p.x = bf(x); p.w1 = bf(w1); p.b1 = b1.data_ptr<float>(); p.w2 = bf(w2); p.b2 = b2.data_ptr<float>();
  p.out = reinterpret_cast<tc_bf16*>(out.data_ptr());
  p.m = (int32_t)m; p.c = (int32_t)c; p.hidden = (int32_t)hidden; p.ldx = (int32_t)x.stride(0); p.ldo = (int32_t)c;
  p.ln = ln_eps >= 0.0 ? 1 : 0; p.ln_eps = ln_eps >= 0.0 ? (float)ln_eps : 0.f;
  check_rc(tc_ff_geglu_fused(&p, cur_stream()), "tc_ff_geglu_fused");
  return out;
}

Tensor ff_geglu_fused_meta(const Tensor& x, const Tensor&, const Tensor&, const Tensor&, const Tensor&, double) {
  return at::empty({x.size(0), x.size(1)}, x.options());
}

Tensor temporal_attn_fused_cuda(const Tensor& x, const Tensor& wqkv, const Tensor& bqkv, const Tensor& wo, const Tensor& bo, int64_t b,
                                int64_t t, int64_t hw, int64_t heads, double ln_eps, double scale) {
  check_rows(x, "temporal_attn_fused: x");
  check_w(wqkv, at::kBFloat16, "temporal_attn_fused: wqkv"); check_w(wo, at::kBFloat16, "temporal_attn_fused: wo");
  check_w(bqkv, at::kFloat, "temporal_attn_fused: bqkv"); check_w(bo, at::kFloat, "temporal_attn_fused: bo");
  const int64_t m = x.size(0), c = x.size(1);
  TORCH_CHECK(m == b * t * hw && wqkv.dim() == 2 && wqkv.size(0) == 3 * c && wqkv.size(1) == c && wo.dim() == 2 && wo.size(0) == c &&
              wo.size(1) == c && bqkv.numel() == 3 * c && bo.numel() == c && c == heads * 64,
              "temporal_attn_fused: x [b*t*hw, c] rows, wqkv [3c, c], bqkv [3c], wo [c, c], bo [c], c = heads * 64");
  Tensor out = at::empty({m, c}, x.options());
// ... 61 lines not shown
  TcDdimParams p = {};
  p.x = x.data_ptr<float>(); p.e_cond = e_cond.data_ptr<float>();
  p.e_uncond = e_uncond.has_value() ? e_uncond->data_ptr<float>() : nullptr;
  p.noise = noise.has_value() ? noise->data_ptr<float>() : nullptr;
  p.e_uncond_img = e_uncond_img.has_value() ? e_uncond_img->data_ptr<float>() : nullptr;
  p.x_prev = x_prev.data_ptr<float>(); p.pred_x0 = x0.data_ptr<float>();
  p.b = (int32_t)x.size(0); p.n = x.numel() / x.size(0);
  p.cfg_scale = (float)cfg_scale; p.cfg_img = (float)cfg_img; p.guidance_rescale = (float)guidance_rescale;
  p.sqrt_ac = (float)sqrt_ac; p.sqrt_1m_ac = (float)sqrt_1m_ac; p.sqrt_a_prev = (float)sqrt_a_prev;
  p.dir_coef = (float)dir_coef; p.sigma = (float)sigma; p.x0_rescale = (float)x0_rescale;
  const int64_t nbytes = tc_ddim_workspace(p.b);
  Tensor ws = at::empty({nbytes > 16 ? nbytes : 16}, x.options().dtype(at::kByte));
  if (EPS)
    check_rc(tc_ddim_step_eps(&p, ws.data_ptr(), nbytes, cur_stream()), "tc_ddim_step_eps");
  else
    check_rc(tc_ddim_step(&p, ws.data_ptr(), nbytes, cur_stream()), "tc_ddim_step");
  return std::make_tuple(x_prev, x0);
}

std::tuple<Tensor, Tensor> ddim_step_meta(const Tensor& x, const Tensor&, const optional<Tensor>&, const optional<Tensor>&,
                                          const optional<Tensor>&, double, double, double, double, double, double, double, double, double) {
  return std::make_tuple(at::empty_like(x), at::empty_like(x));
}

Tensor ddim_blend_cuda(const optional<Tensor>& x, const Tensor& x0, const optional<Tensor>& noise, const optional<Tensor>& mask,
                       double sqrt_ac, double sqrt_1m_ac) {
  auto ok = [&](const Tensor& t) {
    return t.is_cuda() && t.scalar_type() == at::kFloat && t.is_contiguous() && t.sizes() == x0.sizes();
  };
  TORCH_CHECK(x0.dim() >= 1 && ok(x0) && (!x.has_value() || ok(*x)) && (!noise.has_value() || ok(*noise)) &&
              (!mask.has_value() || ok(*mask)), "ddim_blend: contiguous fp32 CUDA tensors of one shape (B, ...)");
  Tensor out = at::empty_like(x0);
  TcDdimBlendParams p = {};
  p.x = x.has_value() ? x->data_ptr<float>() : nullptr;
  p.x0 = x0.data_ptr<float>();
  p.noise = noise.has_value() ? noise->data_ptr<float>() : nullptr;
  p.mask = mask.has_value() ? mask->data_ptr<float>() : nullptr;
  p.out = out.data_ptr<float>();
  p.b = (int32_t)x0.size(0); p.n = p.b ? x0.numel() / x0.size(0) : 0;
  p.sqrt_ac = (float)sqrt_ac; p.sqrt_1m_ac = (float)sqrt_1m_ac;
  check_rc(tc_ddim_blend(&p, cur_stream()), "tc_ddim_blend");
  return out;
}

Tensor ddim_blend_meta(const optional<Tensor>&, const Tensor& x0, const optional<Tensor>&, const optional<Tensor>&, double, double) {
  return at::empty_like(x0);
}

}

TORCH_LIBRARY(tooncrafter, m) {
  m.def("gemm(Tensor a, Tensor w, Tensor? bias, Tensor? residual, Tensor? row_bias, int row_div, int act, float alpha, "
        "float out_scale, bool out_f32, int[] conv, float a_norm_eps=-1.0) -> Tensor");
  m.def("quant_mxfp8(Tensor x, int k) -> (Tensor, Tensor)");
  m.def("gemm_mx(Tensor aq, Tensor a_scale, Tensor wq, Tensor w_scale, Tensor? bias, Tensor? residual, Tensor? row_bias, "
        "int row_div, int act, float alpha, float out_scale, bool out_f32, int[] conv) -> Tensor");
  m.def("attention(Tensor q, Tensor k, Tensor v, int batch, int heads, int lq, int lk, int kv_bdiv, float scale, "
        "Tensor? k2, Tensor? v2, int lk2, int kv2_bdiv) -> Tensor");
  m.def("attention_temporal(Tensor qkv, int b, int t, int hw, int heads, float scale) -> Tensor");
  m.def("attention_q8(Tensor q, Tensor k, Tensor v, int batch, int heads, int lq, int lk, float scale) -> Tensor");
  m.def("groupnorm(Tensor x, Tensor gamma, Tensor beta, int samples, int rows, float eps, bool silu) -> Tensor");
  m.def("ff_geglu_fused(Tensor x, Tensor w1, Tensor b1, Tensor w2, Tensor b2, float ln_eps) -> Tensor");
  m.def("temporal_attn_fused(Tensor x, Tensor wqkv, Tensor bqkv, Tensor wo, Tensor bo, int b, int t, int hw, int heads, float ln_eps, float scale) -> Tensor");
  m.def("temporal_qkv_attn(Tensor x, Tensor wqkv, Tensor? bqkv, int b, int t, int hw, int heads, float scale) -> Tensor");
  m.def("layernorm(Tensor x, Tensor gamma, Tensor beta, float eps) -> Tensor");
  m.def("groupnorm_pf(Tensor x, Tensor gamma, Tensor beta, int samples, int rows, float eps, bool silu, Tensor[] prefetch) -> Tensor");
  m.def("layernorm_pf(Tensor x, Tensor gamma, Tensor beta, float eps, Tensor[] prefetch) -> Tensor");
  m.def("ddim_step(Tensor x, Tensor e_cond, Tensor? e_uncond, Tensor? noise, Tensor? e_uncond_img, float cfg_scale, "
        "float cfg_img, float guidance_rescale, float sqrt_ac, float sqrt_1m_ac, float sqrt_a_prev, float dir_coef, "
        "float sigma, float x0_rescale) -> (Tensor, Tensor)");
  m.def("ddim_step_eps(Tensor x, Tensor e_cond, Tensor? e_uncond, Tensor? noise, Tensor? e_uncond_img, float cfg_scale, "
        "float cfg_img, float guidance_rescale, float sqrt_ac, float sqrt_1m_ac, float sqrt_a_prev, float dir_coef, "
        "float sigma, float x0_rescale) -> (Tensor, Tensor)");
  m.def("ddim_blend(Tensor? x, Tensor x0, Tensor? noise, Tensor? mask, float sqrt_ac, float sqrt_1m_ac) -> Tensor");
  m.def("abi_version() -> int");
}

TORCH_LIBRARY_IMPL(tooncrafter, CUDA, m) {
  m.impl("gemm", gemm_cuda);
  m.impl("quant_mxfp8", quant_mxfp8_cuda);
  m.impl("gemm_mx", gemm_mx_cuda);
  m.impl("attention", attention_cuda);
  m.impl("attention_temporal", attention_temporal_cuda);
  m.impl("attention_q8", attention_q8_cuda);
  m.impl("groupnorm", groupnorm_cuda);
  m.impl("layernorm", layernorm_cuda);
  m.impl("groupnorm_pf", groupnorm_pf_cuda);
  m.impl("layernorm_pf", layernorm_pf_cuda);
  m.impl("ddim_step", ddim_step_any<false>);
  m.impl("ddim_step_eps", ddim_step_any<true>);
  m.impl("ddim_blend", ddim_blend_cuda);
  m.impl("ff_geglu_fused", ff_geglu_fused_cuda);
  m.impl("temporal_attn_fused", temporal_attn_fused_cuda);
  m.impl("temporal_qkv_attn", temporal_qkv_attn_cuda);
}

TORCH_LIBRARY_IMPL(tooncrafter, Meta, m) {
  m.impl("gemm", gemm_meta);
  m.impl("quant_mxfp8", quant_mxfp8_meta);
  m.impl("gemm_mx", gemm_mx_meta);
  m.impl("attention", attention_meta);
  m.impl("attention_temporal", attention_temporal_meta);
  m.impl("attention_q8", attention_q8_meta);
  m.impl("groupnorm", like_meta3);
  m.impl("layernorm", like_meta_ln);
  m.impl("groupnorm_pf", groupnorm_pf_meta);
  m.impl("layernorm_pf", layernorm_pf_meta);
  m.impl("ddim_step", ddim_step_meta);
  m.impl("ddim_step_eps", ddim_step_meta);
  m.impl("ddim_blend", ddim_blend_meta);
  m.impl("ff_geglu_fused", ff_geglu_fused_meta);
  m.impl("temporal_attn_fused", temporal_attn_fused_meta);
  m.impl("temporal_qkv_attn", temporal_qkv_attn_meta);
}

TORCH_LIBRARY_IMPL(tooncrafter, CompositeExplicitAutograd, m) {
  m.impl("abi_version", []() -> int64_t { return tc_abi_version(); });
}
```

### tooncrafter_amd/lvdm/common.py

```python
from __future__ import annotations

from dataclasses import dataclass

import torch
import torch.nn as nn

from .. import ops

BF16 = torch.bfloat16


def ceil_to(x: int, m: int) -> int:
    return (x + m - 1) // m * m


@dataclass
class Act:
    rows: torch.Tensor
    b: int
    t: int
    h: int
    w: int

    @property
    def frames(self) -> int:
        return self.b * self.t

    @property
    def hw(self) -> int:
        return self.h * self.w

    @property
    def c(self) -> int:
        return self.rows.shape[1]

    def like(self, rows, h=None, w=None) -> "Act":
        return Act(rows, self.b, self.t, self.h if h is None else h, self.w if w is None else w)


class CfgShare:

    def __init__(self, n: int, emb1: torch.Tensor, branches: bool = False):
        self.n, self.emb1, self.done, self.branches = n, emb1, False, branches
        self.embn = emb1 if branches else ops.repeat_rows(emb1, n)
        self.memo, self.replay, self.fork = {}, False, None

    def emb(self) -> torch.Tensor:
        return self.embn if self.done else self.emb1

    def expand(self, act: "Act") -> "Act":
        return Act(ops.repeat_rows(act.rows, self.n), act.b * self.n, act.t, act.h, act.w)

    def begin(self, k: int):
        self.replay, self.done = k > 0, False

    def cached(self, key, fn):
        if not self.branches:
            return fn()
        if self.replay and key in self.memo:
            return self.memo[key]
        v = fn()
        if not self.replay and not self.done:
            self.memo[key] = v
        return v

    def split(self, x: torch.Tensor):
        if self.branches and not self.replay and x.is_cuda:
            self.fork = torch.cuda.current_stream(x.device).record_event()
        self.done = True


class SourceKey:

    def __init__(self, tensors):
        self.tensors = list(tensors)
        self.versions = [None if t is None else t._version for t in self.tensors]

    def same(self, tensors) -> bool:
        tensors = list(tensors)
        if len(tensors) != len(self.tensors):
            return False
        for a, b, v in zip(self.tensors, tensors, self.versions):
            if a is not b or (a is not None and a._version != v):
                return False
        return True


# ... 93 lines not shown
```

### tooncrafter_amd/lvdm/openaimodel3d.py

```python
from __future__ import annotations

from typing import List, Optional

import torch
import torch.nn as nn

from .. import ops
from .._lib import ACT_SILU
from .attention import ContextCache, SpatialTransformer, TemporalTransformer, check_frames
from .common import Act, CfgShare, PackedModule, ceil_to, f32, pack_conv3x3, pack_convt3, pack_linear


def conv_nd(dims, *args, **kwargs):
    return {1: nn.Conv1d, 2: nn.Conv2d, 3: nn.Conv3d}[dims](*args, **kwargs)


def normalization(channels, num_groups=32):
    return nn.GroupNorm(num_groups, channels)


def _conv_geom(act: Act, cin: int, stride=1, upsample=False):
    h_out = act.h * 2 if upsample else (act.h + 2 - 3) // stride + 1
    w_out = act.w * 2 if upsample else (act.w + 2 - 3) // stride + 1
    return dict(kind="3x3", frames=act.frames, cin=cin, h_in=act.h, w_in=act.w, h_out=h_out, w_out=w_out,
# ... 57 lines not shown
            pk[f"g{i}"], pk[f"b{i}"] = f32(seq[0].weight), f32(seq[0].bias)
            pk[f"w{i}"], pk[f"cb{i}"] = pack_convt3(seq[-1].weight), f32(seq[-1].bias)
        return pk

    def forward(self, act: Act, part=None) -> Act:
        pk = self.pk
        y = act.rows
        geom = dict(kind="t3", frames=act.frames, t_len=act.t, cin=act.c, h_out=act.h, w_out=act.w)
        gn = dict(samples=act.b, rows=act.t * act.hw, eps=1e-5, silu=True, conv=geom)
        for i in range(1, 5):
            if i < 4:
                y, part = ops.gn_conv(y, pk[f"g{i}"], pk[f"b{i}"], pk[f"w{i}"], pk[f"cb{i}"], part=part, gn_stats=True, **gn)
            else:
                y = ops.gn_conv(y, pk[f"g{i}"], pk[f"b{i}"], pk[f"w{i}"], pk[f"cb{i}"], part=part, residual=act.rows, **gn)
        return act.like(y)


class ResBlock(TimestepBlock, PackedModule):
    def __init__(self, channels, emb_channels, dropout, out_channels=None, use_scale_shift_norm=False, dims=2,
                 use_checkpoint=False, use_conv=False, up=False, down=False, use_temporal_conv=False,
                 tempspatial_aware=False):
        PackedModule.__init__(self)
        if use_scale_shift_norm or up or down or dims != 2 or use_conv:
            raise NotImplementedError("ResBlock variant unused by the config")
        self.channels = channels
        self.emb_channels = emb_channels
        self.out_channels = out_channels or channels
        self.use_temporal_conv = use_temporal_conv
        self.in_layers = nn.Sequential(normalization(channels), nn.SiLU(), nn.Conv2d(channels, self.out_channels, 3, padding=1))
        self.emb_layers = nn.Sequential(nn.SiLU(), nn.Linear(emb_channels, self.out_channels))
        self.out_layers = nn.Sequential(normalization(self.out_channels), nn.SiLU(), nn.Dropout(p=dropout),
                                        nn.Conv2d(self.out_channels, self.out_channels, 3, padding=1))
        if self.out_channels == channels:
            self.skip_connection = nn.Identity()
        else:
            self.skip_connection = nn.Conv2d(channels, self.out_channels, 1)
        if use_temporal_conv:
            self.temopral_conv = TemporalConvBlock(self.out_channels, self.out_channels, dropout=0.1,
                                                   spatial_aware=tempspatial_aware)
        self.emb_slice = None

    def _pack(self):
        pk = {"g1": f32(self.in_layers[0].weight), "b1": f32(self.in_layers[0].bias),
              "w1": pack_conv3x3(self.in_layers[2].weight), "cb1": f32(self.in_layers[2].bias),
              "g2": f32(self.out_layers[0].weight), "b2": f32(self.out_layers[0].bias),
              "w2": pack_conv3x3(self.out_layers[3].weight), "cb2": f32(self.out_layers[3].bias)}
        if not isinstance(self.skip_connection, nn.Identity):
            pk["ws"], pk["bs"] = pack_linear(self.skip_connection.weight), f32(self.skip_connection.bias)
        return pk

    def forward(self, act: Act, emb_all: torch.Tensor) -> Act:
        pk = self.pk
        off, width = self.emb_slice
        geom1, _, _ = _conv_geom(act, ceil_to(act.c, 64))
        gn = dict(samples=act.frames, rows=act.hw, eps=1e-5, silu=True)
        h, part = ops.gn_conv(act.rows, pk["g1"], pk["b1"], pk["w1"], pk["cb1"], conv=geom1, row_bias=emb_all[:, off:off + width],
                              row_div=act.t * act.hw, gn_stats=True, prefetch_extra=(pk["ws"],) if "ws" in pk else (), **gn)
        skip = act.rows if "ws" not in pk else ops.gemm(act.rows, pk["ws"], pk["bs"])
        geom2, _, _ = _conv_geom(act, self.out_channels)
        if not self.use_temporal_conv:
            return act.like(ops.gn_conv(h, pk["g2"], pk["b2"], pk["w2"], pk["cb2"], conv=geom2, part=part, residual=skip, **gn))
        h, part = ops.gn_conv(h, pk["g2"], pk["b2"], pk["w2"], pk["cb2"], conv=geom2, part=part, residual=skip, gn_stats=True, **gn)
        return self.temopral_conv(act.like(h), part)


class TimestepEmbedSequential(nn.Sequential, TimestepBlock):
    def forward(self, act: Act, emb_all, ctx: Optional[ContextCache] = None, share=None) -> Act:
        for j, layer in enumerate(self):
            def run(layer=layer, act=act):
                if isinstance(layer, ResBlock):
                    return layer(act, emb_all if share is None else share.emb())
                if isinstance(layer, SpatialTransformer):
                    return layer(act, ctx, share if share is not None and not share.done else None)
                return layer(act)
            act = run() if share is None or share.done else share.cached(("layer", id(self), j), run)
        return act


class InputConv(PackedModule):

    def __init__(self, cin, cout):
        super().__init__()
        ref = nn.Conv2d(cin, cout, 3, padding=1)
        self.weight = ref.weight
        self.bias = ref.bias
        self.cin_pad = ceil_to(cin, 64)

    def _pack(self):
        return {"w": pack_conv3x3(self.weight, self.cin_pad), "b": f32(self.bias)}

    def forward(self, act: Act) -> Act:
        geom, _, _ = _conv_geom(act, self.cin_pad)
        return act.like(ops.gemm(act.rows, self.pk["w"], self.pk["b"], conv=geom))


class UNetModel(PackedModule):
    def __init__(self, in_channels, model_channels, out_channels, num_res_blocks, attention_resolutions,
                 dropout=0.0, channel_mult=(1, 2, 4, 8), conv_resample=True, dims=2, context_dim=None,
                 use_scale_shift_norm=False, resblock_updown=False, num_heads=-1, num_head_channels=-1,
                 transformer_depth=1, use_linear=False, use_checkpoint=False, temporal_conv=False,
                 tempspatial_aware=False, temporal_attention=True, use_relative_position=True,
                 use_causal_attention=False, temporal_length=None, use_fp16=False, addition_attention=False,
                 temporal_selfatt_only=True, image_cross_attention=False,
                 image_cross_attention_scale_learnable=False, default_fs=4, fs_condition=False):
        super().__init__()
        if num_head_channels == -1:
            raise NotImplementedError("set num_head_channels (the config uses 64)")
        if resblock_updown or dims != 2 or not conv_resample:
            raise NotImplementedError("UNet variant unused by the config")
        self.in_channels, self.model_channels, self.out_channels = in_channels, model_channels, out_channels
        self.num_res_blocks, self.attention_resolutions = num_res_blocks, attention_resolutions
        self.channel_mult, self.temporal_attention = channel_mult, temporal_attention
        self.addition_attention, self.temporal_length = addition_attention, temporal_length
        self.image_cross_attention, self.default_fs, self.fs_condition = image_cross_attention, default_fs, fs_condition
        self.dtype = torch.float32
        ted = model_channels * 4
        self.time_embed = nn.Sequential(nn.Linear(model_channels, ted), nn.SiLU(), nn.Linear(ted, ted))
        if fs_condition:
            self.fps_embedding = nn.Sequential(nn.Linear(model_channels, ted), nn.SiLU(), nn.Linear(ted, ted))

        def st(ch, heads):
            return SpatialTransformer(ch, heads, num_head_channels, depth=transformer_depth, context_dim=context_dim,
                                      use_linear=use_linear, use_checkpoint=use_checkpoint, disable_self_attn=False,
                                      video_length=temporal_length, image_cross_attention=image_cross_attention,
# ... 93 lines not shown
        pk = self.pk
        mc = self.model_channels
        ted = 4 * mc
        dev = timesteps.device
        def dense(v):
            return (v if v.dtype == torch.int64 else v.to(torch.float32)).contiguous()
        te = ops.timestep_embedding(dense(timesteps), mc, ceil_to(mc, 8))
        hcat = torch.empty((b, 2 * ted if self.fs_condition else ted), dtype=torch.bfloat16, device=dev)
        ops.gemm(te, pk["te_w0"], pk["te_b0"], act=ACT_SILU, out=hcat[:, :ted])
        if self.fs_condition:
            if fs is None:
                fs = torch.full((b,), self.default_fs, dtype=torch.long, device=dev)
            fe = ops.timestep_embedding(dense(fs), mc, ceil_to(mc, 8))
            ops.gemm(fe, pk["fe_w0"], pk["fe_b0"], act=ACT_SILU, out=hcat[:, ted:])
        semb = ops.gemm(hcat, pk["e2_w"], pk["e2_b"], act=ACT_SILU)
        return ops.gemm(semb, pk["emb_w"], pk["emb_b"], out_f32=True)

    def forward(self, x, timesteps, context=None, features_adapter=None, fs=None, x_parts=None, replicas=1,
                branches=False, **kwargs):
        if features_adapter is not None:
            raise NotImplementedError("features_adapter is unused by the inference path")
        parts = x_parts if x_parts is not None else [x]
        b, _, t, hh, ww = parts[0].shape
        check_frames(t)
        if replicas > 1 and (context is None or context.shape[0] != replicas * b):
            raise ValueError(f"replicas={replicas}: context must carry {replicas * b} samples")
        cin_pad = ceil_to(self.in_channels, 64)
        rows = ops.nchw_to_rows(parts[0], parts[1] if len(parts) > 1 else None, c_pad=cin_pad)
        act = Act(rows, b, t, hh, ww)
        ctx = self.context_cache(context, t)
        emb_all = self._embedding(timesteps, fs, b)
        if replicas > 1 and branches:
            return self._forward_branches(act, emb_all, ctx, replicas)
        share = CfgShare(replicas, emb_all) if replicas > 1 else None
        return self._body(act, emb_all, ctx, share)

    def _body(self, act: Act, emb_all, ctx, share: Optional[CfgShare]):
        t = act.t
        hs = []
        for i, module in enumerate(self.input_blocks):
            act = module(act, emb_all, ctx, share)
            if i == 0 and self.addition_attention:
                act = self.init_attn(act, emb_all, ctx, share)
            hs.append(act)
        if share is not None:
            if not share.done:
                raise NotImplementedError("replicas > 1 needs a cross-attention in the input blocks to part the passes at")
            emb_all = share.embn
        act = self.middle_block(act, emb_all, ctx)
        for module in self.output_blocks:
            skip = hs.pop()
            if skip.b != act.b:
                skip = share.expand(skip)
            act = act.like(ops.concat_rows(act.rows, skip.rows))
            act = module(act, emb_all, ctx)
        pk = self.pk
        h = ops.groupnorm(act.rows, pk["og"], pk["ob"], samples=act.frames, rows=act.hw, eps=1e-5, silu=True)
        geom, _, _ = _conv_geom(act, act.c)
        y = ops.gemm(h, pk["ow"], pk["ocb"], conv=geom, out_f32=True)
        return ops.rows_to_nchw(y, c=self.out_channels, b=act.b, t=t, h=act.h, w=act.w)

    def _forward_branches(self, act: Act, emb_all, ctx: ContextCache, n: int):
        if getattr(self, "_cross", None) is None:
            self._cross = [m for m in self.modules() if getattr(m, "is_self", True) is False]
        for m in self._cross:
            m.context_kv(ctx)
        share = CfgShare(n, emb_all, branches=True)
        cuda = act.rows.is_cuda
        main = torch.cuda.current_stream(act.rows.device) if cuda else None
        side = self._side_streams(n - 1, act.rows.device) if cuda else []
        outs = []
        for k in range(n):
            share.begin(k)
            if k == 0 or not cuda:
                outs.append(self._body(act, emb_all, ctx.branch(k, act.b), share))
            else:
                side[k - 1].wait_event(share.fork)
                with torch.cuda.stream(side[k - 1]):
                    outs.append(self._body(act, emb_all, ctx.branch(k, act.b), share))
        for s in side:
            main.wait_stream(s)
        return outs

    def _side_streams(self, n: int, device):
        st = getattr(self, "_streams", None)
        if st is None or len(st) < n or st[0].device != device:
            st = self._streams = [torch.cuda.Stream(device=device) for _ in range(n)]
        return st[:n]
```

### tooncrafter_amd/ops.py

```python
from __future__ import annotations

import contextlib
import ctypes as C
from typing import Optional

import torch

from . import _lib
from ._lib import (ACT_GEGLU, ACT_GELU, ACT_NONE, ACT_SILU, GATHER_CONV3x3, GATHER_CONVT3,
                   GATHER_LINEAR, TcAttnParams, TcAttnQ8Params, TcDdimBlendParams, TcDdimParams, TcFfParams, TcGemmMxParams, TcGemmParams, TcTbParams, TcTqaParams)

BF16 = torch.bfloat16


def _stream() -> int:
    return torch.cuda.current_stream().cuda_stream


def _ptr(t: Optional[torch.Tensor]):
    return None if t is None else t.data_ptr()


def _rows_view(t: torch.Tensor, dtype=BF16):
    if t.dim() != 2 or t.stride(1) != 1 or t.dtype != dtype:
# ... 10 lines not shown
    if not isinstance(t, torch.Tensor) or not t.is_cuda:
        raise _lib.TooncrafterHipError(f"{what}: expected a CUDA tensor, got "
                                       f"{getattr(t, 'device', type(t))}: the product path is GPU-only")
    if t.dtype != dtype:
        raise ValueError(f"{what}: expected {dtype}, got {t.dtype}")
    if contiguous and not t.is_contiguous():
        raise ValueError(f"{what}: must be contiguous")
    return t.data_ptr()


class MxRows:

    def __init__(self, q, scales, k):
        self.q, self.scales, self.k = q, scales, k
        self.shape = (q.shape[0], k)
        self.device = q.device


class GnPart:
    __slots__ = ("sums", "rows", "of")

    def __init__(self, sums, rows, of):
        self.sums, self.rows, self.of = sums, rows, of


class HipOps:

    name = "hip"

    def __init__(self):
        import os
        self.lib = _lib.load()
        self._ws = {}
        mode = os.environ.get("TC_FP8", "0").lower()
        self.fp8 = None if mode in ("0", "", "off") else ("linear" if mode in ("1", "on") else mode)
        self.fp8_min_k = int(os.environ.get("TC_FP8_MIN_K", "640"))
        self.fp8_min_n = int(os.environ.get("TC_FP8_MIN_N", "1280"))
        self.fp8_max_cin = int(os.environ.get("TC_FP8_MAX_CIN", "1280"))
        self.fp8_min_cin = int(os.environ.get("TC_FP8_MIN_CIN", "0"))
        self.fp8_n_over_k = float(os.environ.get("TC_FP8_N_OVER_K", "2"))
        self.fp8_min_m = 1024
        self.fp8_decoder = os.environ.get("TC_FP8_DECODER", "0") == "1"
        self.fp8_fuse_ln = os.environ.get("TC_FP8_FUSE_LN", "1") != "0"
        self.fp8_attn = os.environ.get("TC_FP8_ATTN", "0") == "1"
        self.fp8_attn_min_lk = int(os.environ.get("TC_FP8_ATTN_MIN_LK", "640"))
        self.fp8_calls = {"mx": 0, "bf16": 0, "attn_q8": 0}
        self._wq = {}
        self.fuse_ln = os.environ.get("TC_FUSE_LN", "1") != "0"
        self.gn_part = os.environ.get("TC_GN_PART", "0") == "1"
        self.prefetch_on = os.environ.get("TC_PREFETCH", "1") != "0"
        self.prefetch_max_rows = int(os.environ.get("TC_PREFETCH_MAX_ROWS", "8192"))
        self.prefetch_min_bytes = 1 << 20
        self.prefetch_max_bytes = 96 << 20

    def _workspace(self, nbytes: int, device) -> torch.Tensor:
        return torch.empty(max(int(nbytes), 16), dtype=torch.uint8, device=device)

    def gemm(self, a, w, bias=None, *, act=ACT_NONE, residual=None, row_bias=None, row_div=0,
             alpha=1.0, out_scale=1.0, out=None, out_f32=False, conv=None, batch=1,
             stride_a=0, stride_w=0, stride_c=0, m=None, a_norm_eps=None, gn_stats=False):
        mx_a = a if isinstance(a, MxRows) else None
        if mx_a is not None:
            if conv is not None or out is not None or batch != 1 or self.fp8 is None:
                raise ValueError("gemm: an MXFP8 activation feeds one plain linear GEMM of the fp8 route")
            a = mx_a.q
        else:
            a = _rows_view(a)
        if w.dtype != BF16 or w.dim() != 2 or w.stride(1) != 1:
            raise ValueError("w must be a [N, K] bf16 tensor with unit column stride")
        _dev(w, BF16, "gemm: w", contiguous=False)
        n, k = w.shape
        n_out = n // 2 if act == ACT_GEGLU else n
        p = TcGemmParams()
        if conv is None:
            mm = a.shape[0] if m is None else m
            p.gather = GATHER_LINEAR
            if a.shape[1] < k:
                raise ValueError(f"A has {a.shape[1]} columns, weight K = {k}")
        else:
            kind = conv["kind"]
            p.gather = GATHER_CONV3x3 if kind == "3x3" else GATHER_CONVT3
            p.cin = conv["cin"]
            p.frames = conv["frames"]
            p.t_len = conv.get("t_len", 1)
            p.h_out, p.w_out = conv["h_out"], conv["w_out"]
            p.h_in, p.w_in = conv.get("h_in", conv["h_out"]), conv.get("w_in", conv["w_out"])
            p.stride = conv.get("stride", 1)
            p.upsample = 1 if conv.get("upsample", False) else 0
            p.pad = conv.get("pad", 1)
            mm = p.frames * p.h_out * p.w_out
            need_rows = p.frames * p.h_in * p.w_in
            if a.shape[0] < need_rows:
                raise ValueError(f"conv source has {a.shape[0]} rows, geometry needs {need_rows}")
            if a.shape[1] < p.cin or k != (9 if kind == "3x3" else 3) * p.cin:
                raise ValueError(f"conv source has {a.shape[1]} channels / weight K = {k}, geometry says cin = {p.cin}")
        if out is None:
            out = torch.empty((mm, n_out), dtype=torch.float32 if out_f32 else BF16, device=a.device)
        else:
            _rows_view(out, torch.float32 if out_f32 else BF16)
            if out.shape[0] < mm or out.shape[1] != n_out:
                raise ValueError(f"out shape {tuple(out.shape)} != ({mm}, {n_out})")
        p.a, p.w, p.c = a.data_ptr(), w.data_ptr(), out.data_ptr()
        if bias is not None:
            if bias.numel() != n:
                raise ValueError("bias must be fp32 [N]")
            p.bias = _dev(bias, torch.float32, "gemm: bias")
        if row_bias is not None:
            if row_bias.dtype != torch.float32 or row_bias.dim() != 2 or row_bias.stride(1) != 1 \
                    or row_bias.shape[1] != n:
                raise ValueError("row_bias must be fp32 [R, N] with unit column stride")
            if row_div <= 0 or row_bias.shape[0] * row_div < mm:
                raise ValueError("row_bias / row_div do not cover M")
            p.row_bias = _dev(row_bias, torch.float32, "gemm: row_bias", contiguous=False)
            p.ldrb = row_bias.stride(0)
        if residual is not None:
            _rows_view(residual)
            if residual.shape[1] != n_out or residual.shape[0] < mm:
                raise ValueError("residual shape mismatch")
            p.residual = residual.data_ptr()
            p.ldr = residual.stride(0)
        p.m, p.n, p.k = mm, n, k
        p.lda, p.ldw, p.ldc = a.stride(0), w.stride(0), out.stride(0)
        p.row_div = row_div
        p.alpha, p.out_scale = float(alpha), float(out_scale)
        p.act, p.out_f32 = act, 1 if out_f32 else 0
        p.batch = batch
        p.stride_a, p.stride_w, p.stride_c = stride_a, stride_w, stride_c
        if a_norm_eps is not None:
            p.a_norm, p.a_norm_eps = 1, float(a_norm_eps)
            if mx_a is not None or self.fp8 is not None and self._fp8_eligible(p, conv is not None, n_out, batch):
                raise ValueError("gemm: a_norm_eps and the MXFP8 route exclude each other")
            if not self.lib.tc_gemm_ws_eligible(C.byref(p)):
                raise ValueError("gemm: a_norm_eps needs a problem the weight-stationary kernel takes (gemm_ln_eligible)")
        if self.fp8 is not None:
            if self._fp8_eligible(p, conv is not None, n_out, batch):
                self.fp8_calls["mx"] += 1
                self._gemm_mx(p, a, w, mx_a)
                return (out, None) if gn_stats else out
            if mx_a is not None:
                raise ValueError("gemm: MXFP8 activation handed to a GEMM the fp8 route does not take")
            self.fp8_calls["bf16"] += 1
        nbytes = self.lib.tc_gemm_workspace(C.byref(p))
        if nbytes > 0:
            ws = self._workspace(nbytes, a.device)
            p.workspace, p.workspace_bytes = ws.data_ptr(), nbytes
        part = None
        if gn_stats and self.gn_part and out.is_contiguous():
            prow = self.lib.tc_gemm_gn_rows(C.byref(p))
            if prow > 0:
                part = GnPart(torch.empty(((mm + prow - 1) // prow, 2, n), dtype=torch.float32, device=a.device), prow, out)
                p.gn_part = part.sums.data_ptr()
        _lib.check(self.lib.tc_gemm_bf16(C.byref(p), _stream()), "tc_gemm_bf16")
        return (out, part) if gn_stats else out

    def gemm_ln_eligible(self, m, n, k, *, geglu=False, lda=None) -> bool:
        if not self.fuse_ln:
            return False
        p = TcGemmParams()
        p.gather, p.m, p.n, p.k = GATHER_LINEAR, int(m), int(n), int(k)
        p.lda, p.ldw = int(lda if lda is not None else k), int(k)
        p.act = ACT_GEGLU if geglu else ACT_NONE
        p.ldc = p.ldr = n // 2 if geglu else n
        p.alpha, p.out_scale, p.batch = 1.0, 1.0, 1
        if not self.lib.tc_gemm_ws_eligible(C.byref(p)):
            return False
        return not (self.fp8 is not None and self._fp8_eligible(p, False, p.ldc, 1))

    def _ff_params(self, m, c, hidden, ldx, ldo, ln_eps):
        p = TcFfParams()
        p.m, p.c, p.hidden, p.ldx, p.ldo = int(m), int(c), int(hidden), int(ldx), int(ldo)
        p.ln, p.ln_eps = (0, 0.0) if ln_eps is None else (1, float(ln_eps))
        return p

    def ff_fused_eligible(self, m, c, hidden, *, ldx=None) -> bool:
        if self.fp8 is not None:
            return False
        p = self._ff_params(m, c, hidden, c if ldx is None else ldx, c, 1e-5)
        return bool(self.lib.tc_ff_geglu_fused_eligible(C.byref(p)))

    def ff_geglu_fused(self, x, w1, b1, w2, b2, *, ln_eps=None):
        m, c = x.shape
        hidden = w2.shape[1]
        _dev(x, BF16, "ff_geglu_fused x", contiguous=False)
        for t, dt, what in ((w1, BF16, "w1"), (w2, BF16, "w2"), (b1, torch.float32, "b1"), (b2, torch.float32, "b2")):
            _dev(t, dt, "ff_geglu_fused " + what)
        if x.stride(1) != 1 or tuple(w1.shape) != (2 * hidden, c) or tuple(w2.shape) != (c, hidden) or b1.numel() != 2 * hidden \
                or b2.numel() != c:
            raise ValueError("ff_geglu_fused: x [m, c] rows, w1 [2 hidden, c], b1 [2 hidden], w2 [c, hidden], b2 [c]")
        out = torch.empty((m, c), dtype=BF16, device=x.device)
        p = self._ff_params(m, c, hidden, x.stride(0), c, ln_eps)
        p.x, p.w1, p.b1, p.w2, p.b2, p.out = (x.data_ptr(), w1.data_ptr(), b1.data_ptr(), w2.data_ptr(), b2.data_ptr(),
                                              out.data_ptr())
        _lib.check(self.lib.tc_ff_geglu_fused(C.byref(p), _stream()), "tc_ff_geglu_fused")
        return out

    def _tb_params(self, b, t, hw, c, heads, ldx, ldo, ln_eps, scale):
        p = TcTbParams()
        p.b, p.t, p.hw, p.c, p.heads, p.ldx, p.ldo = int(b), int(t), int(hw), int(c), int(heads), int(ldx), int(ldo)
        p.ln, p.ln_eps = (0, 0.0) if ln_eps is None else (1, float(ln_eps))
        p.scale = float(64 ** -0.5 if scale is None else scale)
        return p

    def temporal_attn_fused_eligible(self, *, b, t, hw, c, heads, ldx=None) -> bool:
        if self.fp8 is not None:
            return False
        p = self._tb_params(b, t, hw, c, heads, c if ldx is None else ldx, c, 1e-5, None)
# ... 161 lines not shown
        p = self._q8_params(q, k, v, out, batch, heads, lq, lk, scale)
        ws = self._workspace(self.lib.tc_attn_q8_workspace(C.byref(p)), q.device)
        p.workspace, p.workspace_bytes = ws.data_ptr(), ws.numel()
        _lib.check(self.lib.tc_attn_q8_quant_kv(C.byref(p), _stream()), "tc_attn_q8_quant_kv")
        _lib.check(self.lib.tc_attn_d64_q8(C.byref(p), _stream()), "tc_attn_d64_q8")
        self.fp8_calls["attn_q8"] += 1
        return out

    def attention_temporal(self, qkv, *, b, t, hw, heads, scale=None):
        qkv = _rows_view(qkv)
        cdim = heads * 64
        if not qkv.is_contiguous() or qkv.shape != (b * t * hw, 3 * cdim):
            raise ValueError("attention_temporal: qkv must be contiguous [b*t*hw, 3*C]")
        out = torch.empty((b * t * hw, cdim), dtype=BF16, device=qkv.device)
        _lib.check(self.lib.tc_attn_temporal(qkv.data_ptr(), out.data_ptr(), b, t, hw, heads,
                                             float(scale if scale is not None else 64 ** -0.5), _stream()),
                   "tc_attn_temporal")
        return out

    def prefetch_list(self, x_rows: int, tensors, linear: bool = False):
        if not self.prefetch_on or not tensors or x_rows > self.prefetch_max_rows:
            return []
        if self.fp8 is not None and not linear and self.fp8 != "linear":
            return []
        out, total = [], 0
        for t in tensors:
            if t is None or not isinstance(t, torch.Tensor) or not t.is_contiguous() or t.data_ptr() % 16:
                continue
            if self.fp8 is not None and linear and t.dim() == 2:
                probe = TcGemmParams()
                probe.m, probe.n, probe.k, probe.gather = x_rows, t.shape[0], t.shape[1], GATHER_LINEAR
                if self._fp8_eligible(probe, False, t.shape[0], 1) or self._fp8_eligible(probe, False, t.shape[0] // 2, 1):
                    continue
            nbytes = t.numel() * t.element_size()
            if nbytes < self.prefetch_min_bytes or total + nbytes > self.prefetch_max_bytes:
                continue
            out.append(t)
            total += nbytes
            if len(out) == _lib.TC_PREFETCH_MAX:
                break
        return out

    @staticmethod
    def _prefetch_struct(tensors):
        pf = _lib.TcPrefetch()
        for i, t in enumerate(tensors):
            if not t.is_cuda:
                raise _lib.TooncrafterHipError("prefetch: a CPU tensor in a norm's prefetch list: the product path is GPU-only")
            pf.ptr[i], pf.bytes[i] = t.data_ptr(), t.numel() * t.element_size()
        pf.n = len(tensors)
        return pf

    def groupnorm(self, x, gamma, beta, *, samples, rows, eps, silu=False, part=None, prefetch=None, prefetch_linear=False):
        x = _rows_view(x)
        c = x.shape[1]
        if not x.is_contiguous() or x.shape[0] != samples * rows:
            raise ValueError("groupnorm: x must be contiguous [samples*rows, C]")
        if gamma.numel() != c or beta.numel() != c:
            raise ValueError("groupnorm: gamma/beta must have C elements")
        gp, bp = _dev(gamma, torch.float32, "groupnorm: gamma"), _dev(beta, torch.float32, "groupnorm: beta")
        y = torch.empty_like(x)
        nbytes = self.lib.tc_groupnorm_workspace(samples, rows, c)
        ws = self._workspace(nbytes, x.device)
        if part is not None and part.of is x and rows % part.rows == 0 and part.sums.shape[2] == c \
                and part.sums.shape[0] * part.rows == samples * rows:
            _lib.check(self.lib.tc_groupnorm_part(x.data_ptr(), y.data_ptr(), gp, bp, part.sums.data_ptr(), part.rows, samples,
                                                  rows, c, float(eps), 1 if silu else 0, ws.data_ptr(), nbytes, _stream()),
                       "tc_groupnorm_part")
            return y
        pfl = self.prefetch_list(x.shape[0], prefetch, linear=prefetch_linear)
        if pfl:
            pf = self._prefetch_struct(pfl)
            _lib.check(self.lib.tc_groupnorm_pf(x.data_ptr(), y.data_ptr(), gp, bp, samples, rows, c, float(eps), 1 if silu else 0,
                                                ws.data_ptr(), nbytes, C.byref(pf), _stream()), "tc_groupnorm_pf")
            return y
        _lib.check(self.lib.tc_groupnorm(x.data_ptr(), y.data_ptr(), gp, bp, samples,
                                         rows, c, float(eps), 1 if silu else 0, ws.data_ptr(), nbytes, _stream()),
                   "tc_groupnorm")
        return y

    def gn_conv(self, x, gamma, beta, w, bias=None, *, samples, rows, eps, conv, silu=True, part=None, prefetch_extra=(), **kw):
        h = self.groupnorm(x, gamma, beta, samples=samples, rows=rows, eps=eps, silu=silu, part=part,
                           prefetch=[w, *prefetch_extra])
        return self.gemm(h, w, bias, conv=conv, **kw)

    def layernorm(self, x, gamma, beta, eps=1e-5, mx_for=None, prefetch=None):
        x = _rows_view(x)
        if not x.is_contiguous():
            raise ValueError("layernorm: x must be contiguous")
        if gamma.numel() != x.shape[1] or beta.numel() != x.shape[1]:
            raise ValueError("layernorm: gamma/beta must have C elements")
        gp, bp = _dev(gamma, torch.float32, "layernorm: gamma"), _dev(beta, torch.float32, "layernorm: beta")
        if mx_for is not None and self.fp8 is not None and self.fp8_fuse_ln:
            probe = TcGemmParams()
            probe.m, probe.n, probe.k, probe.gather = x.shape[0], mx_for[0], x.shape[1], GATHER_LINEAR
            if self._fp8_eligible(probe, False, mx_for[1], 1):
                rows, k = x.shape
                lds = (k + 127) // 128 * 4
                q = torch.empty((rows, k), dtype=torch.uint8, device=x.device)
                sc = torch.empty((rows, lds), dtype=torch.uint8, device=x.device)
                _lib.check(self.lib.tc_layernorm_mxfp8(x.data_ptr(), q.data_ptr(), k, sc.data_ptr(), lds, gp, bp, rows, k,
                                                       float(eps), _stream()), "tc_layernorm_mxfp8")
                return MxRows(q, sc, k)
        y = torch.empty_like(x)
        pfl = self.prefetch_list(x.shape[0], prefetch, linear=True)
        if pfl:
            pf = self._prefetch_struct(pfl)
            _lib.check(self.lib.tc_layernorm_pf(x.data_ptr(), y.data_ptr(), gp, bp, x.shape[0], x.shape[1], float(eps),
                                                C.byref(pf), _stream()), "tc_layernorm_pf")
            return y
        _lib.check(self.lib.tc_layernorm(x.data_ptr(), y.data_ptr(), gp, bp,
                                         x.shape[0], x.shape[1], float(eps), _stream()), "tc_layernorm")
        return y

    def softmax_rows(self, s, n=None, causal_period=0):
        if s.dtype != torch.float32 or s.dim() != 2 or not s.is_contiguous() or not s.is_cuda:
            raise ValueError("softmax_rows: contiguous fp32 CUDA [rows, n]")
        ld = s.shape[1]
        n = ld if n is None else int(n)
        p = torch.empty(s.shape, dtype=BF16, device=s.device)
        _lib.check(self.lib.tc_softmax_rows(s.data_ptr(), p.data_ptr(), s.shape[0], n, ld, ld, ld,
                                            int(causal_period), _stream()), "tc_softmax_rows")
        return p

    def nchw_to_rows(self, x0, x1=None, *, c_pad, scale=1.0, out=None):
        if x0.dtype != torch.float32 or x0.dim() != 5 or not x0.is_cuda:
            raise ValueError("nchw_to_rows: fp32 CUDA (B, C, T, H, W)")
        x0 = x0.contiguous()
        b, c0, t, h, w = x0.shape
        c1 = 0
        if x1 is not None:
# ... 184 lines not shown
```

### tooncrafter_amd/torch_ops.py

```python
from __future__ import annotations

import os

import torch

from . import _lib
from ._lib import ACT_NONE
from .ops import HipOps

HERE = os.path.dirname(os.path.abspath(__file__))
LIB_PATH = os.path.join(HERE, "libtooncrafter_torch.so")
_loaded = False


def load():
    global _loaded
    if _loaded:
        return torch.ops.tooncrafter
    if not os.path.exists(LIB_PATH):
        raise _lib.TooncrafterHipError(f"{LIB_PATH} not found: build it with `python -m tooncrafter_amd.build`")
    torch.ops.load_library(LIB_PATH)
    got = int(torch.ops.tooncrafter.abi_version())
    if got != _lib.TC_ABI_VERSION:
        raise _lib.TooncrafterAbiError(f"{LIB_PATH} was built against ABI {got}, this tree is ABI {_lib.TC_ABI_VERSION}: "
                                       "rebuild with `python -m tooncrafter_amd.build`")
    _loaded = True
    return torch.ops.tooncrafter


def conv_list(conv):
    if conv is None:
        return []
    return [1 if conv["kind"] == "3x3" else 2, conv["cin"], conv["frames"], conv.get("t_len", 1),
            conv.get("h_in", conv["h_out"]), conv.get("w_in", conv["w_out"]), conv["h_out"], conv["w_out"],
            conv.get("stride", 1), 1 if conv.get("upsample", False) else 0, conv.get("pad", 1)]


class TorchLibOps(HipOps):

    name = "hip"
    binding = "torch"

    def __init__(self):
        super().__init__()
        self.t = load()

    def gemm(self, a, w, bias=None, *, act=ACT_NONE, residual=None, row_bias=None, row_div=0, alpha=1.0, out_scale=1.0,
             out=None, out_f32=False, conv=None, batch=1, stride_a=0, stride_w=0, stride_c=0, m=None, a_norm_eps=None,
             gn_stats=False):
        if out is not None or batch != 1 or m is not None or self.fp8 is not None or (gn_stats and self.gn_part):
            return super().gemm(a, w, bias, act=act, residual=residual, row_bias=row_bias, row_div=row_div, alpha=alpha,
                                out_scale=out_scale, out=out, out_f32=out_f32, conv=conv, batch=batch, stride_a=stride_a,
                                stride_w=stride_w, stride_c=stride_c, m=m, a_norm_eps=a_norm_eps, gn_stats=gn_stats)
        res = self.t.gemm(a, w, bias, residual, row_bias, int(row_div), int(act), float(alpha), float(out_scale),
                          bool(out_f32), conv_list(conv), -1.0 if a_norm_eps is None else float(a_norm_eps))
        return (res, None) if gn_stats else res

    def quant_mxfp8(self, x, k=None):
        return self.t.quant_mxfp8(x, int(x.shape[1] if k is None else k))

    def attention(self, q, k, v, *, batch, heads, lq, lk, kv_bdiv=1, out=None, accumulate=False, scale=None,
                  k2=None, v2=None, lk2=0, kv2_bdiv=1):
        if out is not None or accumulate:
            return super().attention(q, k, v, batch=batch, heads=heads, lq=lq, lk=lk, kv_bdiv=kv_bdiv, out=out,
                                     accumulate=accumulate, scale=scale, k2=k2, v2=v2, lk2=lk2, kv2_bdiv=kv2_bdiv)
        return self.t.attention(q, k, v, batch, heads, lq, lk, kv_bdiv, float(64 ** -0.5 if scale is None else scale),
                                k2, v2, int(lk2), int(kv2_bdiv))

    def attention_q8(self, q, k, v, *, batch, heads, lq, lk, scale=None):
        out = self.t.attention_q8(q, k, v, int(batch), int(heads), int(lq), int(lk), float(64 ** -0.5 if scale is None else scale))
        self.fp8_calls["attn_q8"] += 1
        return out

    def attention_temporal(self, qkv, *, b, t, hw, heads, scale=None):
        return self.t.attention_temporal(qkv, b, t, hw, heads, float(64 ** -0.5 if scale is None else scale))

    def ff_geglu_fused(self, x, w1, b1, w2, b2, *, ln_eps=None):
        return self.t.ff_geglu_fused(x, w1, b1, w2, b2, -1.0 if ln_eps is None else float(ln_eps))

    def temporal_attn_fused(self, x, wqkv, bqkv, wo, bo, *, b, t, hw, heads, ln_eps=None, scale=None):
        return self.t.temporal_attn_fused(x, wqkv, bqkv, wo, bo, int(b), int(t), int(hw), int(heads),
                                          -1.0 if ln_eps is None else float(ln_eps), float(64 ** -0.5 if scale is None else scale))

    def temporal_qkv_attn(self, x, wqkv, bqkv=None, *, b, t, hw, heads, scale=None, out=None):
        if out is not None:
            return super().temporal_qkv_attn(x, wqkv, bqkv, b=b, t=t, hw=hw, heads=heads, scale=scale, out=out)
        return self.t.temporal_qkv_attn(x, wqkv, bqkv, int(b), int(t), int(hw), int(heads), float(64 ** -0.5 if scale is None else scale))

    def groupnorm(self, x, gamma, beta, *, samples, rows, eps, silu=False, part=None, prefetch=None, prefetch_linear=False):
        if part is not None:
            return super().groupnorm(x, gamma, beta, samples=samples, rows=rows, eps=eps, silu=silu, part=part, prefetch=prefetch,
                                     prefetch_linear=prefetch_linear)
        pfl = self.prefetch_list(x.shape[0], prefetch, linear=prefetch_linear)
        if pfl:
            return self.t.groupnorm_pf(x, gamma, beta, samples, rows, float(eps), bool(silu), pfl)
        return self.t.groupnorm(x, gamma, beta, samples, rows, float(eps), bool(silu))

    def layernorm(self, x, gamma, beta, eps=1e-5, mx_for=None, prefetch=None):
        if mx_for is not None and self.fp8 is not None:
            return super().layernorm(x, gamma, beta, eps, mx_for=mx_for, prefetch=prefetch)
        pfl = self.prefetch_list(x.shape[0], prefetch, linear=True)
        if pfl:
            return self.t.layernorm_pf(x, gamma, beta, float(eps), pfl)
        return self.t.layernorm(x, gamma, beta, float(eps))

    def ddim_step(self, x, e_cond, e_uncond, noise, *, cfg_scale, guidance_rescale, sqrt_ac, sqrt_1m_ac, sqrt_a_prev,
                  dir_coef, sigma, x0_rescale, want_x0=True, e_uncond_img=None, cfg_img=None, parameterization="v"):
        if parameterization not in ("v", "eps"):
            raise NotImplementedError(f"ddim_step: parameterization {parameterization!r} (the fused step has 'v' and 'eps')")
        op = self.t.ddim_step if parameterization == "v" else self.t.ddim_step_eps
        xp, x0 = op(x, e_cond, e_uncond, noise, e_uncond_img, float(cfg_scale),
                    float(cfg_scale if cfg_img is None else cfg_img), float(guidance_rescale), float(sqrt_ac),
                    float(sqrt_1m_ac), float(sqrt_a_prev), float(dir_coef), float(sigma), float(x0_rescale))
        return xp, (x0 if want_x0 else None)

    def ddim_blend(self, x, x0, noise, mask, *, sqrt_ac=1.0, sqrt_1m_ac=0.0, out=None):
        if out is not None:
            return super().ddim_blend(x, x0, noise, mask, sqrt_ac=sqrt_ac, sqrt_1m_ac=sqrt_1m_ac, out=out)
        return self.t.ddim_blend(x, x0, noise, mask, float(sqrt_ac), float(sqrt_1m_ac))
```

Before: 8.413 frames/s.

## Read UNet skip concatenation from two sources in GEMM and GroupNorm

```diff
diff --git a/include/tooncrafter_hip.h b/include/tooncrafter_hip.h
--- a/include/tooncrafter_hip.h
+++ b/include/tooncrafter_hip.h
@@ -57,12 +57,15 @@
   int32_t a_norm;
   float a_norm_eps;
   float* gn_part;
+  const tc_bf16* a2;
+  int32_t lda2, k_split;
 } TcGemmParams;
 
 int tc_gemm_bf16(const TcGemmParams* p, void* stream);
 int64_t tc_gemm_workspace(const TcGemmParams* p);
 int tc_gemm_ws_eligible(const TcGemmParams* p);
 int tc_gemm_gn_rows(const TcGemmParams* p);
+int tc_gemm_pair_ok(const TcGemmParams* p);
 
 typedef struct TcGemmMxParams {
   TcGemmParams g;
@@ -157,6 +160,11 @@
 int tc_layernorm_pf(const tc_bf16* x, tc_bf16* y, const float* gamma, const float* beta,
                     int32_t rows, int32_t c, float eps, const TcPrefetch* prefetch, void* stream);
 
+int tc_groupnorm_pair(const tc_bf16* x, int32_t ldx, const tc_bf16* x2, int32_t ldx2, int32_t c1, tc_bf16* y,
+                      const float* gamma, const float* beta, int32_t samples, int32_t rows, int32_t c, float eps,
+                      int32_t silu, void* workspace, int64_t workspace_bytes, const TcPrefetch* prefetch,
+                      void* stream);
+
 int tc_softmax_rows(const float* s, tc_bf16* p, int32_t rows, int32_t n, int32_t n_out, int32_t lds, int32_t ldo,
                     int32_t causal_period, void* stream);
 
diff --git a/tooncrafter_amd/_lib.py b/tooncrafter_amd/_lib.py
--- a/tooncrafter_amd/_lib.py
+++ b/tooncrafter_amd/_lib.py
@@ -32,6 +32,7 @@
         ("workspace", C.c_void_p), ("workspace_bytes", C.c_int64),
         ("a_norm", C.c_int32), ("a_norm_eps", C.c_float),
         ("gn_part", C.c_void_p),
+        ("a2", C.c_void_p), ("lda2", C.c_int32), ("k_split", C.c_int32),
     ]
 
 
@@ -159,6 +160,10 @@
     "tc_ddim_blend": (C.c_int, [C.POINTER(TcDdimBlendParams), C.c_void_p]),
     "tc_gemm_ws_eligible": (C.c_int, [C.POINTER(TcGemmParams)]),
     "tc_gemm_gn_rows": (C.c_int, [C.POINTER(TcGemmParams)]),
+    "tc_gemm_pair_ok": (C.c_int, [C.POINTER(TcGemmParams)]),
+    "tc_groupnorm_pair": (C.c_int, [C.c_void_p, C.c_int32, C.c_void_p, C.c_int32, C.c_int32, C.c_void_p, C.c_void_p, C.c_void_p,
+                                    C.c_int32, C.c_int32, C.c_int32, C.c_float, C.c_int32, C.c_void_p, C.c_int64,
+                                    C.POINTER(TcPrefetch), C.c_void_p]),
     "tc_groupnorm_part": (C.c_int, [C.c_void_p, C.c_void_p, C.c_void_p, C.c_void_p, C.c_void_p, C.c_int32, C.c_int32, C.c_int32,
                                     C.c_int32, C.c_float, C.c_int32, C.c_void_p, C.c_int64, C.c_void_p]),
     "tc_ff_geglu_fused_eligible": (C.c_int, [C.POINTER(TcFfParams)]),
diff --git a/tooncrafter_amd/csrc/gemm.hip b/tooncrafter_amd/csrc/gemm.hip
--- a/tooncrafter_amd/csrc/gemm.hip
+++ b/tooncrafter_amd/csrc/gemm.hip
@@ -7,7 +7,7 @@
 
 constexpr int BK = TC_BK;
 
-template <int GATHER, int TM, int TN, bool PIPE>
+template <int GATHER, int TM, int TN, bool PIPE, bool TWO = false>
 __global__ __launch_bounds__(256, 2) void gemm_kernel(const TcGemmParams pin, const int splits, const int order,
                                                       const int late_epi) {
   TcGemmParams p = pin;
@@ -44,7 +44,18 @@
   const int chunk = (tid & 7) ^ ((lrow >> 1) & 7);
   AGather<GATHER, RA> ag;
   ag.init(p, tile_m * BM, lrow, 32, chunk);
-  const tc_rsrc_t a_rsrc = tc_a_rsrc(p, bz, ag.row_lo);
+  const tc_rsrc_t a_rsrc = !TWO ? tc_a_rsrc(p, bz, ag.row_lo)
+                                : make_rsrc(reinterpret_cast<const bf16_t*>(p.a) + ag.row_lo * p.lda,
+                                            (((int64_t)p.m - 1 - ag.row_lo) * p.lda + p.k_split) * 2);
+  const tc_rsrc_t a2_rsrc = !TWO ? a_rsrc
+                                 : make_rsrc(reinterpret_cast<const bf16_t*>(p.a2) + ag.row_lo * p.lda2,
+                                             (((int64_t)p.m - 1 - ag.row_lo) * p.lda2 + (p.k - p.k_split)) * 2);
+  uint32_t a2_base[TWO ? RA : 1];
+  if (TWO) {
+#pragma unroll
+    for (int i = 0; i < RA; ++i)
+      a2_base[i] = ag.ok[i] ? (uint32_t)(((int64_t)(tile_m * BM + lrow + 32 * i) - ag.row_lo) * p.lda2 * 2 + chunk * 16) : TC_OOB;
+  }
   uint32_t b_voff[RB];
 #pragma unroll
   for (int i = 0; i < RB; ++i) {
@@ -69,6 +80,12 @@
 #pragma unroll
     for (int i = 0; i < RB; ++i)
       glds16(w_rsrc, sb + i * 4096, b_voff[i] | kill, (uint32_t)k0 * 2u);
+    if (TWO && k0 >= p.k_split) {
+#pragma unroll
+      for (int i = 0; i < RA; ++i)
+        glds16(a2_rsrc, sa + i * 4096, a2_base[i] | kill, (uint32_t)(k0 - p.k_split) * 2u);
+      return;
+    }
 #pragma unroll
     for (int i = 0; i < RA; ++i)
       glds16(a_rsrc, sa + i * 4096, a_voff[i] | kill, a_soff);
@@ -258,6 +275,17 @@
     else if (r.tn == 2) hipLaunchKernelGGL((gemm_kernel<G, 1, 2, P>), grid, block, 0, s, p, r.splits, r.order, r.late_epi);
     else hipLaunchKernelGGL((gemm_kernel<G, 1, 1, P>), grid, block, 0, s, p, r.splits, r.order, r.late_epi);
   };
+  if (p.a2) {
+    const auto go2 = [&](auto pipe) {
+      constexpr int G = TC_GATHER_LINEAR, P = decltype(pipe)::value;
+      if (r.tm == 2 && r.tn == 2) hipLaunchKernelGGL((gemm_kernel<G, 2, 2, P, true>), grid, block, 0, s, p, r.splits, r.order, r.late_epi);
+      else if (r.tm == 2) hipLaunchKernelGGL((gemm_kernel<G, 2, 1, P, true>), grid, block, 0, s, p, r.splits, r.order, r.late_epi);
+      else if (r.tn == 2) hipLaunchKernelGGL((gemm_kernel<G, 1, 2, P, true>), grid, block, 0, s, p, r.splits, r.order, r.late_epi);
+      else hipLaunchKernelGGL((gemm_kernel<G, 1, 1, P, true>), grid, block, 0, s, p, r.splits, r.order, r.late_epi);
+    };
+    if (r.pipe) go2(std::true_type{}); else go2(std::false_type{});
+    return;
+  }
   tc_with_gather(p.gather, [&](auto g) { if (r.pipe) go(g, std::true_type{}); else go(g, std::false_type{}); });
 }
 
diff --git a/tooncrafter_amd/csrc/gemm_mx.hip b/tooncrafter_amd/csrc/gemm_mx.hip
--- a/tooncrafter_amd/csrc/gemm_mx.hip
+++ b/tooncrafter_amd/csrc/gemm_mx.hip
@@ -324,7 +324,7 @@
   if ((reinterpret_cast<uintptr_t>(pp->a_scale) & 1u) || (reinterpret_cast<uintptr_t>(pp->w_scale) & 3u)) return TC_EALIGN;
   if ((pp->lda_s & 1) || (pp->ldw_s & 3)) return TC_EALIGN;
   if (p.ldw < p.k || pp->ldw_s < ((p.k + 127) / 128) * 4) return TC_ESHAPE;
-  if ((p.batch > 1) || p.stride_a || p.stride_w || p.stride_c) return TC_ESHAPE;
+  if ((p.batch > 1) || p.stride_a || p.stride_w || p.stride_c || p.a2) return TC_ESHAPE;
   const bool geglu = p.act == TC_ACT_GEGLU;
   const int n_out = geglu ? p.n / 2 : p.n;
   if ((n_out & 7) == 0) {
diff --git a/tooncrafter_amd/csrc/gemm_route.cpp b/tooncrafter_amd/csrc/gemm_route.cpp
--- a/tooncrafter_amd/csrc/gemm_route.cpp
+++ b/tooncrafter_amd/csrc/gemm_route.cpp
@@ -84,7 +84,13 @@
   if (geglu && ((p.n % 128) != 0 || p.row_bias || p.residual)) return TC_ESHAPE;
   if (p.row_bias && (p.row_div <= 0 || p.ldrb < p.n)) return TC_EINVAL;
   if (p.act < TC_ACT_NONE || p.act > TC_ACT_GEGLU) return TC_EINVAL;
-  if (p.gather == TC_GATHER_LINEAR) {
+  if (p.a2) {
+    if (p.gather != TC_GATHER_LINEAR || p.batch > 1 || p.a_norm) return TC_ESHAPE;
+    if (p.k_split <= 0 || p.k_split >= p.k || (p.k_split % TC_BK) != 0) return TC_ESHAPE;
+    if (p.lda < p.k_split || p.lda2 < p.k - p.k_split) return TC_ESHAPE;
+    if (!aligned16(p.a2) || (p.lda2 & 7)) return TC_EALIGN;
+    if ((int64_t)257 * p.lda2 * 2 >= 0x7fffff00LL) return TC_ESHAPE;
+  } else if (p.gather == TC_GATHER_LINEAR) {
     if (p.lda < p.k) return TC_ESHAPE;
   } else if (p.gather == TC_GATHER_CONV3x3 || p.gather == TC_GATHER_CONVT3) {
     const int taps = p.gather == TC_GATHER_CONV3x3 ? 9 : 3;
@@ -324,6 +330,13 @@
 }
 
 int tc_gemm_route(const TcGemmParams& p, const TcGemmSwitches& sw, int cus, TcGemmRoute* r) {
+  if (p.a2) {
+    TcGemmParams q = p;
+    q.a2 = nullptr, q.lda2 = 0, q.k_split = 0, q.lda = p.k;
+    const int rc = tc_gemm_route(q, sw, cus, r);
+    if (rc != TC_OK) return rc;
+    return r->family == TC_FAM_TILE ? TC_OK : TC_ESHAPE;
+  }
   *r = TcGemmRoute{};
   const int batch = p.batch > 0 ? p.batch : 1;
   const bool gn_ok = batch == 1 && p.act != TC_ACT_GEGLU && !p.out_f32 && (p.n & 7) == 0 && !p.a_norm && !sw.tile_set && sw.gn_part;
@@ -355,6 +368,12 @@
   return (p && tc_gemm_ws_takes(*p, tc_gemm_switches(), p->batch > 0 ? p->batch : 1)) ? 1 : 0;
 }
 
+extern "C" int tc_gemm_pair_ok(const TcGemmParams* p) {
+  if (!p || !p->a2 || tc_gemm_validate(*p) != TC_OK) return 0;
+  TcGemmRoute r;
+  return tc_gemm_route(*p, tc_gemm_switches(), 256, &r) == TC_OK ? 1 : 0;
+}
+
 extern "C" int tc_gemm_gn_rows(const TcGemmParams* pp) {
   if (!pp || pp->m <= 0 || pp->n <= 0 || pp->k <= 0) return 0;
   TcGemmParams p = *pp;
diff --git a/tooncrafter_amd/csrc/norm.hip b/tooncrafter_amd/csrc/norm.hip
--- a/tooncrafter_amd/csrc/norm.hip
+++ b/tooncrafter_amd/csrc/norm.hip
@@ -41,6 +41,16 @@
   }
 }
 
+struct GnSrc {
+  const bf16_t* x; const bf16_t* x2;
+  int c1, ld, ld2;
+};
+__device__ __forceinline__ const bf16_t* gn_src_vec(const GnSrc& s, int64_t row0, int ch, int& ld) {
+  if (ch < s.c1) { ld = s.ld; return s.x + row0 * s.ld + ch; }
+  ld = s.ld2;
+  return s.x2 + row0 * s.ld2 + (ch - s.c1);
+}
+
 struct GnGeo {
   int vpr;
   int slots;
@@ -73,7 +83,7 @@
   }
 }
 
-__global__ __launch_bounds__(GN_THREADS) void gn_stats_kernel(const bf16_t* __restrict__ x, float* __restrict__ part,
+__global__ __launch_bounds__(GN_THREADS) void gn_stats_kernel(const GnSrc src, float* __restrict__ part,
                                                               int rows, int c, int nchunks, int chunk_rows) {
   __shared__ float red[2][4096 + 32];
   const GnGeo g = gn_geo(c);
@@ -83,7 +93,10 @@
   const int sample = blockIdx.y, chunk = blockIdx.x;
   const int r0 = chunk * chunk_rows;
   const int r1 = min(rows, r0 + chunk_rows);
-  const bf16_t* xs = x + (int64_t)sample * rows * c;
+  const bf16_t* xs[GN_MAX_SLOTS];
+  int ldx[GN_MAX_SLOTS];
+#pragma unroll
+  for (int s = 0; s < GN_MAX_SLOTS; ++s) xs[s] = gn_src_vec(src, (int64_t)sample * rows, vec[s] >= 0 ? vec[s] * 8 : 0, ldx[s]);
 
   float sum[GN_MAX_SLOTS][8], sq[GN_MAX_SLOTS][8];
 #pragma unroll
@@ -100,7 +113,7 @@
 #pragma unroll
         for (int u = 0; u < 4; ++u) {
           const int rr = r + u * step;
-          v4[u] = rr < r1 ? *reinterpret_cast<const u32x4*>(xs + (int64_t)rr * c + vec[s] * 8)
+          v4[u] = rr < r1 ? *reinterpret_cast<const u32x4*>(xs[s] + (int64_t)rr * ldx[s])
                           : u32x4{0u, 0u, 0u, 0u};
         }
 #pragma unroll
@@ -193,7 +206,7 @@
 }
 
 template <bool SILU>
-__global__ __launch_bounds__(GN_THREADS) void gn_apply_kernel(const bf16_t* __restrict__ x, bf16_t* __restrict__ y,
+__global__ __launch_bounds__(GN_THREADS) void gn_apply_kernel(const GnSrc src, bf16_t* __restrict__ y,
                                                               const float* __restrict__ gamma, const float* __restrict__ beta,
                                                               const float* __restrict__ stats, int rows, int c,
                                                               int chunk_rows, const PfArgs pf) {
@@ -225,7 +238,10 @@
     }
   const int r0 = chunk * chunk_rows;
   const int r1 = min(rows, r0 + chunk_rows);
-  const bf16_t* xs = x + (int64_t)sample * rows * c;
+  const bf16_t* xs[GN_MAX_SLOTS];
+  int ldx[GN_MAX_SLOTS];
+#pragma unroll
+  for (int s = 0; s < GN_MAX_SLOTS; ++s) xs[s] = gn_src_vec(src, (int64_t)sample * rows, vec[s] >= 0 ? vec[s] * 8 : 0, ldx[s]);
   bf16_t* ys = y + (int64_t)sample * rows * c;
   const int step = g.rows_pp;
   for (int r = r0 + rlane; r < r1; r += 4 * step) {
@@ -236,7 +252,7 @@
 #pragma unroll
         for (int u = 0; u < 4; ++u) {
           const int rr = r + u * step;
-          if (rr < r1) v4[u] = *reinterpret_cast<const u32x4*>(xs + (int64_t)rr * c + vec[s] * 8);
+          if (rr < r1) v4[u] = *reinterpret_cast<const u32x4*>(xs[s] + (int64_t)rr * ldx[s]);
         }
 #pragma unroll
         for (int u = 0; u < 4; ++u) {
@@ -260,7 +276,7 @@
 __device__ __forceinline__ void gn_opaque(u32x4& v) { asm volatile("" : "+v"(v[0]), "+v"(v[1]), "+v"(v[2]), "+v"(v[3])); }
 
 template <int T, int NV, bool SILU>
-__global__ __launch_bounds__(T) void gn_onepass_kernel(const bf16_t* __restrict__ x, bf16_t* __restrict__ y,
+__global__ __launch_bounds__(T) void gn_onepass_kernel(const GnSrc src, bf16_t* __restrict__ y,
                                                        const float* __restrict__ gamma, const float* __restrict__ beta,
                                                        int rows, int c, int vu, float eps, const PfArgs pf) {
   if (blockIdx.z) {
@@ -278,7 +294,8 @@
   const int unit = blockIdx.x, sample = blockIdx.y;
   const int ch0 = (unit * vu + col) * 8;
   const int ug0 = (unit * vu * 8) / cpg;
-  const bf16_t* xs = x + (int64_t)sample * rows * c + ch0;
+  int ldx;
+  const bf16_t* xs = gn_src_vec(src, (int64_t)sample * rows, ch0, ldx);
   bf16_t* ys = y + (int64_t)sample * rows * c + ch0;
   int gl[8];
 #pragma unroll
@@ -288,7 +305,7 @@
 #pragma unroll
   for (int i = 0; i < NV; ++i) {
     const int r = r0 + i * rpp;
-    v[i] = (live && r < rows) ? *reinterpret_cast<const u32x4*>(xs + (int64_t)r * c) : u32x4{0u, 0u, 0u, 0u};
+    v[i] = (live && r < rows) ? *reinterpret_cast<const u32x4*>(xs + (int64_t)r * ldx) : u32x4{0u, 0u, 0u, 0u};
   }
   auto group_sums = [&](const float (&pc)[8], int slot, float (&out)[4]) {
     float g4[4] = {0.f, 0.f, 0.f, 0.f};
@@ -549,6 +566,13 @@
   return ((int64_t)samples * nch * 64 + (int64_t)samples * 64) * sizeof(float);
 }
 
+static int gn_check2(const tc_bf16* x2, int32_t ldx, int32_t ldx2, int32_t c1, int32_t c) {
+  if (!x2) return (c1 == c && ldx >= c && (ldx & 7) == 0) ? TC_OK : (ldx < c ? TC_ESHAPE : TC_EALIGN);
+  if (c1 <= 0 || c1 >= c || (c1 & 7) || ldx < c1 || ldx2 < c - c1) return TC_ESHAPE;
+  if ((ldx & 7) || (ldx2 & 7) || !tc_aligned16(x2)) return TC_EALIGN;
+  return TC_OK;
+}
+
 static int gn_check(const tc_bf16* x, tc_bf16* y, const float* gamma, const float* beta, int32_t samples, int32_t rows,
                     int32_t c, void* workspace, int64_t workspace_bytes, const TcPrefetch* prefetch, PfArgs* pf) {
   if (!x || !y || !gamma || !beta || !workspace || samples <= 0 || rows <= 0 || c <= 0) return TC_EINVAL;
@@ -561,7 +585,7 @@
 }
 
 struct GnIo {
-  const bf16_t* x; bf16_t* y; const float* gamma; const float* beta;
+  GnSrc x; bf16_t* y; const float* gamma; const float* beta;
   int rows, c; bool silu; hipStream_t s;
 };
 static void gn_apply_launch(const GnIo& io, dim3 grid, const float* stats, int chunk_rows, const PfArgs& pf) {
@@ -574,13 +598,15 @@
   hipLaunchKernelGGL(k, grid, dim3(T), 0, io.s, io.x, io.y, io.gamma, io.beta, io.rows, io.c, vu, eps, pf);
 }
 
-static int groupnorm_impl(const tc_bf16* x, tc_bf16* y, const float* gamma, const float* beta,
+static int groupnorm_impl(const tc_bf16* x, int32_t ldx, const tc_bf16* x2, int32_t ldx2, int32_t c1, tc_bf16* y,
+                          const float* gamma, const float* beta,
                           int32_t samples, int32_t rows, int32_t c, float eps, int32_t silu,
                           void* workspace, int64_t workspace_bytes, const TcPrefetch* prefetch, void* stream) {
   PfArgs pf;
   if (const int rc = gn_check(x, y, gamma, beta, samples, rows, c, workspace, workspace_bytes, prefetch, &pf)) return rc;
-  const GnIo io = {reinterpret_cast<const bf16_t*>(x), reinterpret_cast<bf16_t*>(y), gamma, beta, rows, c, silu != 0,
-                   reinterpret_cast<hipStream_t>(stream)};
+  if (const int rc = gn_check2(x2, ldx, ldx2, c1, c)) return rc;
+  const GnIo io = {GnSrc{reinterpret_cast<const bf16_t*>(x), reinterpret_cast<const bf16_t*>(x2), c1, ldx, ldx2},
+                   reinterpret_cast<bf16_t*>(y), gamma, beta, rows, c, silu != 0, reinterpret_cast<hipStream_t>(stream)};
   {
     static const bool onepass = [] { const char* e = getenv("TC_GN_ONEPASS"); return !(e && e[0] == '0'); }();
     const int cpg = c / 32;
@@ -621,13 +647,21 @@
 extern "C" int tc_groupnorm(const tc_bf16* x, tc_bf16* y, const float* gamma, const float* beta,
                             int32_t samples, int32_t rows, int32_t c, float eps, int32_t silu,
                             void* workspace, int64_t workspace_bytes, void* stream) {
-  return groupnorm_impl(x, y, gamma, beta, samples, rows, c, eps, silu, workspace, workspace_bytes, nullptr, stream);
+  return groupnorm_impl(x, c, nullptr, 0, c, y, gamma, beta, samples, rows, c, eps, silu, workspace, workspace_bytes, nullptr, stream);
 }
 
 extern "C" int tc_groupnorm_pf(const tc_bf16* x, tc_bf16* y, const float* gamma, const float* beta,
                                int32_t samples, int32_t rows, int32_t c, float eps, int32_t silu,
                                void* workspace, int64_t workspace_bytes, const TcPrefetch* prefetch, void* stream) {
-  return groupnorm_impl(x, y, gamma, beta, samples, rows, c, eps, silu, workspace, workspace_bytes, prefetch, stream);
+  return groupnorm_impl(x, c, nullptr, 0, c, y, gamma, beta, samples, rows, c, eps, silu, workspace, workspace_bytes, prefetch, stream);
+}
+
+extern "C" int tc_groupnorm_pair(const tc_bf16* x, int32_t ldx, const tc_bf16* x2, int32_t ldx2, int32_t c1, tc_bf16* y,
+                                 const float* gamma, const float* beta, int32_t samples, int32_t rows, int32_t c, float eps,
+                                 int32_t silu, void* workspace, int64_t workspace_bytes, const TcPrefetch* prefetch,
+                                 void* stream) {
+  if (!x2) return TC_EINVAL;
+  return groupnorm_impl(x, ldx, x2, ldx2, c1, y, gamma, beta, samples, rows, c, eps, silu, workspace, workspace_bytes, prefetch, stream);
 }
 
 extern "C" int tc_groupnorm_part(const tc_bf16* x, tc_bf16* y, const float* gamma, const float* beta, const float* part,
@@ -637,8 +671,8 @@
   PfArgs pf;
   if (const int rc = gn_check(x, y, gamma, beta, samples, rows, c, workspace, workspace_bytes, nullptr, &pf)) return rc;
   if ((rows % part_rows) != 0) return TC_ESHAPE;
-  const GnIo io = {reinterpret_cast<const bf16_t*>(x), reinterpret_cast<bf16_t*>(y), gamma, beta, rows, c, silu != 0,
-                   reinterpret_cast<hipStream_t>(stream)};
+  const GnIo io = {GnSrc{reinterpret_cast<const bf16_t*>(x), nullptr, c, c, 0}, reinterpret_cast<bf16_t*>(y), gamma, beta, rows, c,
+                   silu != 0, reinterpret_cast<hipStream_t>(stream)};
   int nch, cr;
   gn_chunking(samples, rows, &nch, &cr);
   float* stats = reinterpret_cast<float*>(workspace) + (int64_t)samples * nch * 64;
diff --git a/tooncrafter_amd/csrc/torch_ops.cpp b/tooncrafter_amd/csrc/torch_ops.cpp
--- a/tooncrafter_amd/csrc/torch_ops.cpp
+++ b/tooncrafter_amd/csrc/torch_ops.cpp
@@ -96,6 +96,35 @@
   }
   check_rc(tc_gemm_bf16(&p, cur_stream()), "tc_gemm_bf16");
   return out;
+}
+
+Tensor gemm_pair_cuda(const Tensor& a, const Tensor& a2, const Tensor& w, const optional<Tensor>& bias, const optional<Tensor>& residual,
+                      const optional<Tensor>& row_bias, int64_t row_div, int64_t act, double alpha, double out_scale, bool out_f32) {
+  check_rows(a, "gemm_pair: a");
+  check_rows(a2, "gemm_pair: a2");
+  check_rows(w, "gemm_pair: w");
+  TORCH_CHECK(a.size(0) == a2.size(0) && a.size(1) + a2.size(1) == w.size(1), "gemm_pair: a [M, K1] and a2 [M, K2] with K1 + K2 = the weight's K");
+  const GemmGeom g = gemm_geom(a, w, act, {});
+  Tensor out = at::empty({g.m, g.n_out}, a.options().dtype(out_f32 ? at::kFloat : at::kBFloat16));
+  TcGemmParams p = {};
+  p.a = bf(a); p.w = bf(w);
+  p.lda = (int32_t)a.stride(0); p.ldw = (int32_t)w.stride(0);
+  p.a2 = bf(a2); p.lda2 = (int32_t)a2.stride(0); p.k_split = (int32_t)a.size(1);
+  fill_gemm(p, w, g, out, bias, residual, row_bias, row_div, act, alpha, out_scale, out_f32, {});
+  Tensor ws;
+  const int64_t nbytes = tc_gemm_workspace(&p);
+  if (nbytes > 0) {
+    ws = at::empty({nbytes}, a.options().dtype(at::kByte));
+    p.workspace = ws.data_ptr(); p.workspace_bytes = nbytes;
+  }
+  check_rc(tc_gemm_bf16(&p, cur_stream()), "tc_gemm_bf16 (two-source)");
+  return out;
+}
+
+Tensor gemm_pair_meta(const Tensor& a, const Tensor&, const Tensor& w, const optional<Tensor>&, const optional<Tensor>&,
+                      const optional<Tensor>&, int64_t, int64_t act, double, double, bool out_f32) {
+  const GemmGeom g = gemm_geom(a, w, act, {});
+  return at::empty({g.m, g.n_out}, a.options().dtype(out_f32 ? at::kFloat : at::kBFloat16));
 }
 
 std::tuple<Tensor, Tensor> quant_mxfp8_cuda(const Tensor& x, int64_t k) {
@@ -263,6 +292,27 @@
                            (int32_t)samples, (int32_t)rows, (int32_t)c, (float)eps, silu ? 1 : 0, ws.data_ptr(), nbytes, &pf, cur_stream()),
            "tc_groupnorm_pf");
   return y;
+}
+
+Tensor groupnorm_pair_cuda(const Tensor& x, const Tensor& x2, const Tensor& gamma, const Tensor& beta, int64_t samples, int64_t rows,
+                           double eps, bool silu, at::TensorList prefetch) {
+  check_rows(x, "groupnorm_pair: x");
+  check_rows(x2, "groupnorm_pair: x2");
+  const int64_t c1 = x.size(1), c = c1 + x2.size(1);
+  TORCH_CHECK(x.size(0) == samples * rows && x2.size(0) == samples * rows, "groupnorm_pair: x and x2 must have samples*rows rows");
+  check_affine(gamma, beta, c, "groupnorm_pair");
+  const TcPrefetch pf = prefetch_of(prefetch, "groupnorm_pair");
+  Tensor y = at::empty({samples * rows, c}, x.options());
+  const int64_t nbytes = tc_groupnorm_workspace((int32_t)samples, (int32_t)rows, (int32_t)c);
+  Tensor ws = at::empty({nbytes > 16 ? nbytes : 16}, x.options().dtype(at::kByte));
+  check_rc(tc_groupnorm_pair(bf(x), (int32_t)x.stride(0), bf(x2), (int32_t)x2.stride(0), (int32_t)c1, reinterpret_cast<tc_bf16*>(y.data_ptr()),
+                             gamma.data_ptr<float>(), beta.data_ptr<float>(), (int32_t)samples, (int32_t)rows, (int32_t)c, (float)eps,
+                             silu ? 1 : 0, ws.data_ptr(), nbytes, &pf, cur_stream()), "tc_groupnorm_pair");
+  return y;
+}
+
+Tensor groupnorm_pair_meta(const Tensor& x, const Tensor& x2, const Tensor&, const Tensor&, int64_t, int64_t, double, bool, at::TensorList) {
+  return at::empty({x.size(0), x.size(1) + x2.size(1)}, x.options());
 }
 
 Tensor layernorm_pf_cuda(const Tensor& x, const Tensor& gamma, const Tensor& beta, double eps, at::TensorList prefetch) {
@@ -430,6 +480,9 @@
 TORCH_LIBRARY(tooncrafter, m) {
   m.def("gemm(Tensor a, Tensor w, Tensor? bias, Tensor? residual, Tensor? row_bias, int row_div, int act, float alpha, "
         "float out_scale, bool out_f32, int[] conv, float a_norm_eps=-1.0) -> Tensor");
+  m.def("gemm_pair(Tensor a, Tensor a2, Tensor w, Tensor? bias, Tensor? residual, Tensor? row_bias, int row_div, int act, float alpha, "
+        "float out_scale, bool out_f32) -> Tensor");
+  m.def("groupnorm_pair(Tensor x, Tensor x2, Tensor gamma, Tensor beta, int samples, int rows, float eps, bool silu, Tensor[] prefetch) -> Tensor");
   m.def("quant_mxfp8(Tensor x, int k) -> (Tensor, Tensor)");
   m.def("gemm_mx(Tensor aq, Tensor a_scale, Tensor wq, Tensor w_scale, Tensor? bias, Tensor? residual, Tensor? row_bias, "
         "int row_div, int act, float alpha, float out_scale, bool out_f32, int[] conv) -> Tensor");
@@ -456,6 +509,8 @@
 
 TORCH_LIBRARY_IMPL(tooncrafter, CUDA, m) {
   m.impl("gemm", gemm_cuda);
+  m.impl("gemm_pair", gemm_pair_cuda);
+  m.impl("groupnorm_pair", groupnorm_pair_cuda);
   m.impl("quant_mxfp8", quant_mxfp8_cuda);
   m.impl("gemm_mx", gemm_mx_cuda);
   m.impl("attention", attention_cuda);
@@ -475,6 +530,8 @@
 
 TORCH_LIBRARY_IMPL(tooncrafter, Meta, m) {
   m.impl("gemm", gemm_meta);
+  m.impl("gemm_pair", gemm_pair_meta);
+  m.impl("groupnorm_pair", groupnorm_pair_meta);
   m.impl("quant_mxfp8", quant_mxfp8_meta);
   m.impl("gemm_mx", gemm_mx_meta);
   m.impl("attention", attention_meta);
diff --git a/tooncrafter_amd/lvdm/common.py b/tooncrafter_amd/lvdm/common.py
--- a/tooncrafter_amd/lvdm/common.py
+++ b/tooncrafter_amd/lvdm/common.py
@@ -1,6 +1,7 @@
 from __future__ import annotations
 
 from dataclasses import dataclass
+from typing import Optional
 
 import torch
 import torch.nn as nn
@@ -21,6 +22,7 @@
     t: int
     h: int
     w: int
+    rows2: Optional[torch.Tensor] = None
 
     @property
     def frames(self) -> int:
@@ -32,7 +34,10 @@
 
     @property
     def c(self) -> int:
-        return self.rows.shape[1]
+        return self.rows.shape[1] + (0 if self.rows2 is None else self.rows2.shape[1])
+
+    def joined(self) -> "Act":
+        return self if self.rows2 is None else self.like(ops.concat_rows(self.rows, self.rows2))
 
     def like(self, rows, h=None, w=None) -> "Act":
         return Act(rows, self.b, self.t, self.h if h is None else h, self.w if w is None else w)
diff --git a/tooncrafter_amd/lvdm/openaimodel3d.py b/tooncrafter_amd/lvdm/openaimodel3d.py
--- a/tooncrafter_amd/lvdm/openaimodel3d.py
+++ b/tooncrafter_amd/lvdm/openaimodel3d.py
@@ -133,11 +133,16 @@
     def forward(self, act: Act, emb_all: torch.Tensor) -> Act:
         pk = self.pk
         off, width = self.emb_slice
+        if act.rows2 is not None:
+            pair_ok = getattr(ops.backend(), "rows_pair_ok", None)
+            if "ws" not in pk or pair_ok is None or not pair_ok(act.rows, act.rows2, pk["ws"], pk["bs"]):
+                act = act.joined()
+        x = act.rows if act.rows2 is None else (act.rows, act.rows2)
         geom1, _, _ = _conv_geom(act, ceil_to(act.c, 64))
         gn = dict(samples=act.frames, rows=act.hw, eps=1e-5, silu=True)
-        h, part = ops.gn_conv(act.rows, pk["g1"], pk["b1"], pk["w1"], pk["cb1"], conv=geom1, row_bias=emb_all[:, off:off + width],
+        h, part = ops.gn_conv(x, pk["g1"], pk["b1"], pk["w1"], pk["cb1"], conv=geom1, row_bias=emb_all[:, off:off + width],
                               row_div=act.t * act.hw, gn_stats=True, prefetch_extra=(pk["ws"],) if "ws" in pk else (), **gn)
-        skip = act.rows if "ws" not in pk else ops.gemm(act.rows, pk["ws"], pk["bs"])
+        skip = x if "ws" not in pk else ops.gemm(x, pk["ws"], pk["bs"])
         geom2, _, _ = _conv_geom(act, self.out_channels)
         if not self.use_temporal_conv:
             return act.like(ops.gn_conv(h, pk["g2"], pk["b2"], pk["w2"], pk["cb2"], conv=geom2, part=part, residual=skip, **gn))
@@ -151,6 +156,7 @@
             def run(layer=layer, act=act):
                 if isinstance(layer, ResBlock):
                     return layer(act, emb_all if share is None else share.emb())
+                act = act.joined()
                 if isinstance(layer, SpatialTransformer):
                     return layer(act, ctx, share if share is not None and not share.done else None)
                 return layer(act)
@@ -350,8 +356,7 @@
             skip = hs.pop()
             if skip.b != act.b:
                 skip = share.expand(skip)
-            act = act.like(ops.concat_rows(act.rows, skip.rows))
-            act = module(act, emb_all, ctx)
+            act = module(Act(act.rows, act.b, act.t, act.h, act.w, rows2=skip.rows), emb_all, ctx)
         pk = self.pk
         h = ops.groupnorm(act.rows, pk["og"], pk["ob"], samples=act.frames, rows=act.hw, eps=1e-5, silu=True)
         geom, _, _ = _conv_geom(act, act.c)
diff --git a/tooncrafter_amd/ops.py b/tooncrafter_amd/ops.py
--- a/tooncrafter_amd/ops.py
+++ b/tooncrafter_amd/ops.py
@@ -86,6 +86,7 @@
         self.prefetch_max_rows = int(os.environ.get("TC_PREFETCH_MAX_ROWS", "8192"))
         self.prefetch_min_bytes = 1 << 20
         self.prefetch_max_bytes = 96 << 20
+        self.two_source = os.environ.get("TC_TWO_SOURCE", "1") != "0"
 
     def _workspace(self, nbytes: int, device) -> torch.Tensor:
         return torch.empty(max(int(nbytes), 16), dtype=torch.uint8, device=device)
@@ -93,6 +94,12 @@
     def gemm(self, a, w, bias=None, *, act=ACT_NONE, residual=None, row_bias=None, row_div=0,
              alpha=1.0, out_scale=1.0, out=None, out_f32=False, conv=None, batch=1,
              stride_a=0, stride_w=0, stride_c=0, m=None, a_norm_eps=None, gn_stats=False):
+        a2 = None
+        if isinstance(a, (tuple, list)):
+            a, a2 = a
+            a2 = _rows_view(a2)
+            if conv is not None or out is not None or batch != 1 or m is not None or a_norm_eps is not None or gn_stats and self.gn_part:
+                raise ValueError("gemm: two-source rows feed one plain linear GEMM")
         mx_a = a if isinstance(a, MxRows) else None
         if mx_a is not None:
             if conv is not None or out is not None or batch != 1 or self.fp8 is None:
@@ -109,7 +116,11 @@
         if conv is None:
             mm = a.shape[0] if m is None else m
             p.gather = GATHER_LINEAR
-            if a.shape[1] < k:
+            if a2 is not None:
+                if a2.shape[0] != a.shape[0] or a.shape[1] + a2.shape[1] != k:
+                    raise ValueError(f"two-source A has {a.shape[1]} + {a2.shape[1]} columns, weight K = {k}")
+                p.a2, p.lda2, p.k_split = a2.data_ptr(), a2.stride(0), a.shape[1]
+            elif a.shape[1] < k:
                 raise ValueError(f"A has {a.shape[1]} columns, weight K = {k}")
         else:
             kind = conv["kind"]
@@ -166,6 +177,8 @@
                 raise ValueError("gemm: a_norm_eps and the MXFP8 route exclude each other")
             if not self.lib.tc_gemm_ws_eligible(C.byref(p)):
                 raise ValueError("gemm: a_norm_eps needs a problem the weight-stationary kernel takes (gemm_ln_eligible)")
+        if a2 is not None and (self.fp8 is not None and self._fp8_eligible(p, False, n_out, 1) or not self.lib.tc_gemm_pair_ok(C.byref(p))):
+            raise ValueError("gemm: this problem does not take two-source rows (ask rows_pair_ok first and concatenate)")
         if self.fp8 is not None:
             if self._fp8_eligible(p, conv is not None, n_out, batch):
                 self.fp8_calls["mx"] += 1
@@ -186,6 +199,22 @@
                 p.gn_part = part.sums.data_ptr()
         _lib.check(self.lib.tc_gemm_bf16(C.byref(p), _stream()), "tc_gemm_bf16")
         return (out, part) if gn_stats else out
+
+    def rows_pair_ok(self, x, x2, w, bias=None) -> bool:
+        if not self.two_source or x.dim() != 2 or x2.dim() != 2 or x.shape[0] != x2.shape[0]:
+            return False
+        c1, c2 = x.shape[1], x2.shape[1]
+        if c1 % 8 or c2 % 8 or (c1 + c2) % 32 or x.stride(1) != 1 or x2.stride(1) != 1 or w.dim() != 2 or w.shape[1] != c1 + c2:
+            return False
+        p = TcGemmParams()
+        p.gather, p.m, p.n, p.k = GATHER_LINEAR, x.shape[0], w.shape[0], w.shape[1]
+        p.a, p.lda, p.a2, p.lda2, p.k_split = x.data_ptr(), x.stride(0), x2.data_ptr(), x2.stride(0), c1
+        p.w, p.ldw, p.c, p.ldc = w.data_ptr(), w.stride(0), w.data_ptr(), w.shape[0]
+        p.bias = _ptr(bias)
+        p.alpha, p.out_scale, p.batch = 1.0, 1.0, 1
+        if self.fp8 is not None and self._fp8_eligible(p, False, p.n, 1):
+            return False
+        return bool(self.lib.tc_gemm_pair_ok(C.byref(p)))
 
     def gemm_ln_eligible(self, m, n, k, *, geglu=False, lda=None) -> bool:
         if not self.fuse_ln:
@@ -453,6 +482,8 @@
         return pf
 
     def groupnorm(self, x, gamma, beta, *, samples, rows, eps, silu=False, part=None, prefetch=None, prefetch_linear=False):
+        if isinstance(x, (tuple, list)):
+            return self._groupnorm_pair(x[0], x[1], gamma, beta, samples, rows, eps, silu, prefetch, prefetch_linear)
         x = _rows_view(x)
         c = x.shape[1]
         if not x.is_contiguous() or x.shape[0] != samples * rows:
@@ -478,6 +509,24 @@
         _lib.check(self.lib.tc_groupnorm(x.data_ptr(), y.data_ptr(), gp, bp, samples,
                                          rows, c, float(eps), 1 if silu else 0, ws.data_ptr(), nbytes, _stream()),
                    "tc_groupnorm")
+        return y
+
+    def _groupnorm_pair(self, x, x2, gamma, beta, samples, rows, eps, silu, prefetch, prefetch_linear):
+        x, x2 = _rows_view(x), _rows_view(x2)
+        c1, c = x.shape[1], x.shape[1] + x2.shape[1]
+        if x.shape[0] != samples * rows or x2.shape[0] != samples * rows:
+            raise ValueError("groupnorm: both sources must have samples*rows rows")
+        if gamma.numel() != c or beta.numel() != c:
+            raise ValueError("groupnorm: gamma/beta must have C elements")
+        gp, bp = _dev(gamma, torch.float32, "groupnorm: gamma"), _dev(beta, torch.float32, "groupnorm: beta")
+        y = torch.empty((samples * rows, c), dtype=BF16, device=x.device)
+        nbytes = self.lib.tc_groupnorm_workspace(samples, rows, c)
+        ws = self._workspace(nbytes, x.device)
+        pfl = self.prefetch_list(x.shape[0], prefetch, linear=prefetch_linear)
+        pf = C.byref(self._prefetch_struct(pfl)) if pfl else None
+        _lib.check(self.lib.tc_groupnorm_pair(x.data_ptr(), x.stride(0), x2.data_ptr(), x2.stride(0), c1, y.data_ptr(), gp, bp,
+                                              samples, rows, c, float(eps), 1 if silu else 0, ws.data_ptr(), nbytes, pf, _stream()),
+                   "tc_groupnorm_pair")
         return y
 
     def gn_conv(self, x, gamma, beta, w, bias=None, *, samples, rows, eps, conv, silu=True, part=None, prefetch_extra=(), **kw):
diff --git a/tooncrafter_amd/torch_ops.py b/tooncrafter_amd/torch_ops.py
--- a/tooncrafter_amd/torch_ops.py
+++ b/tooncrafter_amd/torch_ops.py
@@ -48,7 +48,13 @@
     def gemm(self, a, w, bias=None, *, act=ACT_NONE, residual=None, row_bias=None, row_div=0, alpha=1.0, out_scale=1.0,
              out=None, out_f32=False, conv=None, batch=1, stride_a=0, stride_w=0, stride_c=0, m=None, a_norm_eps=None,
              gn_stats=False):
-        if out is not None or batch != 1 or m is not None or self.fp8 is not None or (gn_stats and self.gn_part):
+        if isinstance(a, (tuple, list)) and self.fp8 is None and not (gn_stats and self.gn_part) and out is None and batch == 1 \
+                and m is None and conv is None and a_norm_eps is None:
+            res = self.t.gemm_pair(a[0], a[1], w, bias, residual, row_bias, int(row_div), int(act), float(alpha), float(out_scale),
+                                   bool(out_f32))
+            return (res, None) if gn_stats else res
+        if out is not None or batch != 1 or m is not None or self.fp8 is not None or (gn_stats and self.gn_part) \
+                or isinstance(a, (tuple, list)):
             return super().gemm(a, w, bias, act=act, residual=residual, row_bias=row_bias, row_div=row_div, alpha=alpha,
                                 out_scale=out_scale, out=out, out_f32=out_f32, conv=conv, batch=batch, stride_a=stride_a,
                                 stride_w=stride_w, stride_c=stride_c, m=m, a_norm_eps=a_norm_eps, gn_stats=gn_stats)
@@ -88,6 +94,9 @@
         return self.t.temporal_qkv_attn(x, wqkv, bqkv, int(b), int(t), int(hw), int(heads), float(64 ** -0.5 if scale is None else scale))
 
     def groupnorm(self, x, gamma, beta, *, samples, rows, eps, silu=False, part=None, prefetch=None, prefetch_linear=False):
+        if isinstance(x, (tuple, list)):
+            pfl = self.prefetch_list(x[0].shape[0], prefetch, linear=prefetch_linear)
+            return self.t.groupnorm_pair(x[0], x[1], gamma, beta, samples, rows, float(eps), bool(silu), pfl)
         if part is not None:
             return super().groupnorm(x, gamma, beta, samples=samples, rows=rows, eps=eps, silu=silu, part=part, prefetch=prefetch,
                                      prefetch_linear=prefetch_linear)
```

After: 8.450 frames/s, median of 6. About the same (+0.4%).
